# NorthStarUAS/ImageAnalysis

Measured on AMD Instinct MI355X. Metric: image_pairs_matched_per_sec, higher is better.
Workload: dtype u8 (int8 MFMA, int32 accumulate)

## Files before the change

### imageanalysis_amd/csrc/match_knn2sym.hip

```cpp
#include "iamx_common.h"
#include "sym_cand_rule.h"

namespace {

typedef int v4i __attribute__((ext_vector_type(4)));
typedef int v2i __attribute__((ext_vector_type(2)));
typedef int v16i __attribute__((ext_vector_type(16)));
typedef unsigned v2u __attribute__((ext_vector_type(2)));

#ifndef IAMX_DESC_OFFSET
#define IAMX_DESC_OFFSET 128
#endif
constexpr int D = IAMX_DESC_DIM;
constexpr int CHUNK = 128;
constexpr int BIG = 0x3F000000;

struct Pack3Args {
    const void *src;
    const int64_t *src_off;
    int64_t single_n;
    const int32_t *dst_off;
    int8_t *dst;
    int32_t *sn2, *sct, *sperm, *sinv;
    int32_t *n2, *nb, *pos;
// ... 650 lines not shown
#pragma unroll
        for (int k = 0; k < 8; ++k) load_op(0, 0, k, aop[0], tbop[0]);
#pragma unroll
        for (int k = 0; k < 8 / PP; ++k) load_op(0, 1, k, aop[1], tbop[1]);
        issue(0, 0, accs[0][0], accs[0][1]);
        __builtin_amdgcn_sched_barrier(0);
        int rbo = 0, rbo_prev = 2 * NW * CHUNK;
        const int wave_u = uniform32(wave);
        typedef __attribute__((address_space(3))) const int8_t *lds_bytes;
        int opoff[4], tboff = 2 * CHUNK * D + 16 * g;
#pragma unroll
        for (int s = 0; s < 4; ++s) opoff[s] = c * D + (((2 * s + g) ^ ((c >> 1) & 7)) * 16);
        auto load_op_at = [&](int tile, int k, v4i (&a)[4], v4i (&tbv)[4]) {
            if (k < 4) tbv[k] = *reinterpret_cast<const __attribute__((address_space(3))) v4i *>((lds_bytes)lds + tboff + tile * 128 + 32 * k);
            else a[k - 4] = *reinterpret_cast<const __attribute__((address_space(3))) v4i *>((lds_bytes)lds + opoff[k - 4] + tile * (32 * D));
        };
        const unsigned stage_voff = (unsigned)((tid >> 3) * D + (((tid & 7) ^ ((tid >> 4) & 7)) * 16));
        const unsigned lds_tile_at = (unsigned)(uintptr_t)(lds_ptr)(lds_tile + wave_u * (64 * 16));
        const unsigned lds_tb_at = (unsigned)(uintptr_t)(lds_ptr)(lds_tb + (wave_u & (CHUNK / 64 - 1)) * 64);
        const unsigned ct_voff = (unsigned)((tid & (CHUNK - 1)) * 4);
#if defined(IAMX_T_STAMPS)
        const unsigned long long loop_c0 = __builtin_amdgcn_s_memtime(), loop_r0 = __builtin_amdgcn_s_memrealtime();
        __builtin_amdgcn_s_waitcnt(0xC07F);
#endif
        for (int ch = 0; ch < nchunks; ++ch) {
            const int buf = ch & 1;
            if constexpr (PP == 4) {
            constexpr int BAR = (NT4 - 1) * PP - 1;
            static_assert(NW == 4 && PIECES == 4 && BAR + 4 < NS && (NT / 8) % 16 == 0, "the gaps below are form 2's");
            const int chs = ch + 2 < nchunks ? ch + 2 : nchunks - 1;
            const int8_t *const sg_tile = tbase + (int64_t)chs * (CHUNK * D);
            const int8_t *const sg_ct = reinterpret_cast<const int8_t *>(tci + chs * CHUNK);
            int mR[NW], mL = BIG, mU1 = BIG, mU2 = BIG;
            static_for<0, NS>([&](auto st_c) {
                constexpr int st = decltype(st_c)::value;
                constexpr int t = st / PP, ph = st % PP, qp = 2 * ph, cur = st & 1;
                constexpr int nst = st + 1 < NS ? st + 1 : 0;
#if defined(IAMX_T_STAMPS)
                unsigned long long stamp_t0 = 0, stamp_t1 = 0;
                if constexpr (IAMX_T_STAMPS == st + 1 || (st == BAR && IAMX_T_STAMPS == 17)) SWEEP_STAMP(stamp_t0);
                if constexpr (st == 0 && IAMX_T_STAMPS == 19) {
                    SWEEP_STAMP(stamp_t0);
                    SWEEP_STAMP(stamp_t1);
                    stamp_sum += stamp_t1 - stamp_t0;
                }
#endif
                if constexpr (st == BAR) {
                    __builtin_amdgcn_s_waitcnt(0x0070);
#if defined(IAMX_T_STAMPS)
                    if constexpr (IAMX_T_STAMPS == 17) {
                        SWEEP_STAMP(stamp_t1);
                        stamp_sum += stamp_t1 - stamp_t0;
                    }
                    if constexpr (IAMX_T_STAMPS == 18) SWEEP_STAMP(stamp_t0);
#endif
                    __syncthreads();
#if defined(IAMX_T_STAMPS)
                    if constexpr (IAMX_T_STAMPS == 18) {
                        SWEEP_STAMP(stamp_t1);
                        stamp_sum += stamp_t1 - stamp_t0;
                    }
#endif
                }
                issue(nst / PP, 2 * (nst % PP), accs[cur ^ 1][0], accs[cur ^ 1][1], false);
                auto operand_reads = [&]() {
                    static_for<(st == BAR - 1 ? 1 : 0), (st == BAR - 2 ? 2 : 1)>([&](auto d_c) {
                        constexpr int sr = st + decltype(d_c)::value;
                        constexpr int T = (sr + 1) / PP + 1, i = (sr + 1) % PP;
#pragma unroll
                        for (int k = i * 8 / PP; k < (i + 1) * 8 / PP; ++k) load_op_at(T % NT4, k, aop[T & 1], tbop[T & 1]);
                    });
                };
                if constexpr (st == BAR) {
#pragma unroll
                    for (int s = 0; s < 4; ++s) opoff[s] ^= CHUNK * D;
                    tboff ^= CHUNK * 4;
                }
                constexpr int nv = (ph == 2 ? 36 : ph == 3 ? 40 : 32) + (st == BAR + 2 ? 11 : 0) + (st == BAR + 3 ? 5 : 0) +
                                   (st >= BAR && st <= BAR + PIECES ? 1 : 0) +
                                   (st == NS - 1 ? 2 : 0);
                constexpr int tail = (st == BAR - 1 ? 0 : st == BAR - 2 ? 4 : 2) + (ph == 3 ? 1 + 2 : 0) +
                                     (st == BAR + 1 ? 2 : 0) + (st == BAR + 3 ? 1 : 0);
                constexpr bool staging = st >= BAR && st <= BAR + PIECES;
                constexpr int STAGE_GAP = 1, STAGE_AT = 8 + 1;
                constexpr int blk_at = sweep_gap_valu(nv, tail, true, 0) + sweep_gap_valu(nv, tail, true, 1) +
                                       sweep_gap_valu(nv, tail, true, 2) - (staging ? 2 : 0);
                static_assert(ph == 3 || (blk_at >= 6 && blk_at < 31), "gaps 3 and 4 hold the last two minima of column chain 0");
                const v16i acc0 = accs[cur][0], acc1 = accs[cur][1];
                int (&rc_)[16] = r[t & 1];
                int (&rp)[16] = r[(t + 1) & 1];
                static_for<0, 32>([&](auto i_c) {
                    constexpr int i = decltype(i_c)::value, op = sweep_min_order(ph < 3, blk_at, i);
                    if constexpr (op < 16) {
                        rc_[op] = qp == 0 ? min(acc0[op], acc1[op]) : min(min(rc_[op], acc0[op]), acc1[op]);
                    } else {
                        constexpr int w = op - 16;
                        int &mm = m[qp + (w >> 3)][t & 3];
                        const v16i &acc = w < 8 ? acc0 : acc1;
                        mm = min(min(mm, acc[2 * (w & 7)]), acc[2 * (w & 7) + 1]);
                        if constexpr (ph < 3 && i == blk_at) row_min16_block<2 * ph, true>(rp, mm);
                        if constexpr (ph < 3 && i == blk_at + 1) row_min16_block<2 * ph + 1, true>(rp, mm);
                        if constexpr (staging && w == STAGE_AT) {
                            if constexpr (st < BAR + PIECES)
                                stage_piece_held<16>(sg_tile + (st - BAR) * ((NT / 8) * D) + stage_voff,
                                                     lds_tile_at + buf * (CHUNK * D) + (st - BAR) * NT * 16, mm);
                            else
                                stage_piece_held<4>(sg_ct + ct_voff, lds_tb_at + buf * (CHUNK * 4), mm);
                        }
                    }
                });
                pin_accs(accs[cur ^ 1][0], accs[cur ^ 1][1]);
                operand_reads();
                if constexpr (ph == 2) {
#pragma unroll
                    for (int k = 0; k < 4; ++k) bu[k] = rp[4 * k] + lo_lane;
                }
                if constexpr (ph == 3) {
                    int *const dst = row_dst + (t > 0 ? rbo : rbo_prev) + (t > 0 ? t - 1 : NT4 - 1) * 32;
                    row_min16_piece<3>(rp, bu, lo_lane, dst);
                }
                if constexpr (st == BAR + 1) {
#pragma unroll
                    for (int w = 0; w < NW; ++w) mR[w] = lds_row[rbo_prev + w * CHUNK + mrow];
                }
                if constexpr (st == BAR + 2) {
#pragma unroll
                    for (int w = 0; w < NW; ++w) {
                        const int uw = mR[w] + spread_w[w];
                        mL = min(mL, mR[w]);
                        mU2 = min(max(mU1, uw), mU2);
                        mU1 = min(mU1, uw);
                    }
                }
                if constexpr (st == BAR + 3)
                    __builtin_amdgcn_raw_buffer_store_b64(v2i{mL, pack_row_bounds(mL, mU1, mU2)}, rowp_rsrc,
                                                          merger && ch > 0 ? ((ch - 1) * CHUNK + mrow) * 8 : RANGE_DROP, 0, 0);
                static_for<0, 8>([&](auto g_c) {
                    constexpr int g = decltype(g_c)::value;
                    __builtin_amdgcn_sched_group_barrier(0x008, 1, 0);
                    __builtin_amdgcn_sched_group_barrier(0x002, sweep_gap_valu(nv, tail, ph < 3, g) + (g == 7 ? 3 : 0) -
                                                                    (staging && g == STAGE_GAP ? 1 : 0), 0);
                });
                __builtin_amdgcn_sched_barrier(0);
#if defined(IAMX_T_STAMPS)
                if constexpr (IAMX_T_STAMPS == st + 1) {
                    SWEEP_STAMP(stamp_t1);
                    stamp_sum += stamp_t1 - stamp_t0;
                }
#endif
            });
            } else {
#pragma unroll
            for (int st = 0; st < NS; ++st) {
                const int t = st / PP, qp = 2 * (st % PP), cur = st & 1;
                if (st == (NT4 - 1) * PP - 1) {
                    __builtin_amdgcn_s_waitcnt(0x0070);
                    __syncthreads();
                    stage_direct(ch + 2 < nchunks ? ch + 2 : nchunks - 1, buf);
                    merge_rows(ch - 1, rbo_prev, merger && ch > 0);
                }
                if (st + 1 < NS) issue((st + 1) / PP, 2 * ((st + 1) % PP), accs[cur ^ 1][0], accs[cur ^ 1][1]);
                else issue(0, 0, accs[cur ^ 1][0], accs[cur ^ 1][1]);
                {
                    const int T = (st + 1) / PP + 1, i = (st + 1) % PP;
#pragma unroll
                    for (int k = i * 8 / PP; k < (i + 1) * 8 / PP; ++k)
                        load_op(T < NT4 ? buf : buf ^ 1, T % NT4, k, aop[T & 1], tbop[T & 1]);
                }
                const v16i acc0 = accs[cur][0], acc1 = accs[cur][1];
                int t0 = min(min(m[qp][t & 3], acc0[0]), acc0[1]);
                int t1m = min(min(m[qp + 1][t & 3], acc1[0]), acc1[1]);
#pragma unroll
                for (int reg = 2; reg < 16; reg += 2) {
                    t0 = min(min(t0, acc0[reg]), acc0[reg + 1]);
                    t1m = min(min(t1m, acc1[reg]), acc1[reg + 1]);
                }
                m[qp][t & 3] = t0;
                m[qp + 1][t & 3] = t1m;
                int (&rc_)[16] = r[t & 1];
                if (qp == 0) {
#pragma unroll
                    for (int reg = 0; reg < 16; ++reg) rc_[reg] = min(acc0[reg], acc1[reg]);
                } else {
#pragma unroll
                    for (int reg = 0; reg < 16; ++reg) rc_[reg] = min(min(rc_[reg], acc0[reg]), acc1[reg]);
                }
                {
                    int (&rp)[16] = r[(t + 1) & 1];
                    const int tp = t > 0 ? t - 1 : NT4 - 1;
                    int *dst = row_dst + (t > 0 ? rbo : rbo_prev) + tp * 32;
                    if constexpr (PP == 1) {
                        int m0, m1;
                        half_wave_min16<true>(rp, lo_lane, m0, m1);
                        dst[0] = m0;
                        dst[16] = m1;
                    } else {
                        if (0 * PP / 4 == st % PP) row_min16_piece<0>(rp, bu, lo_lane, dst);
                        if (1 * PP / 4 == st % PP) row_min16_piece<1>(rp, bu, lo_lane, dst);
                        if (2 * PP / 4 == st % PP) row_min16_piece<2>(rp, bu, lo_lane, dst);
                        if (3 * PP / 4 == st % PP) row_min16_piece<3>(rp, bu, lo_lane, dst);
                    }
                }
#pragma unroll
                for (int i = 0; i < 8; ++i) {
                    __builtin_amdgcn_sched_group_barrier(0x008, 1, 0);
                    __builtin_amdgcn_sched_group_barrier(0x002, PIPE, 0);
                }
                __builtin_amdgcn_sched_barrier(0);
            }
            }
            rbo_prev = rbo;
            rbo = rbo == 2 * NW * CHUNK ? 0 : rbo + NW * CHUNK;
        }
#if defined(IAMX_T_STAMPS)
        if constexpr (PP == 4) {
            unsigned long long loop_c1;
            SWEEP_STAMP(loop_c1);
            stamp_cycles += loop_c1 - loop_c0;
            stamp_ticks += __builtin_amdgcn_s_memrealtime() - loop_r0;
            stamp_chunks += (unsigned)nchunks;
            if (A.stamps && lane == 0) {
                unsigned long long *o = A.stamps + ((size_t)blockIdx.x * NW + wave) * 4;
                o[0] = stamp_sum;
                o[1] = stamp_chunks;
                o[2] = stamp_cycles;
                o[3] = stamp_ticks;
            }
        }
#endif
        int64_t col_v = 0;
        if constexpr (ITEMS) col_v = A.col_off[u];
        {
            int m0, m1;
            half_wave_min16<true>(r[(NT4 - 1) & 1], lo_lane, m0, m1);
            int *dst = row_dst + rbo_prev + (NT4 - 1) * 32;
            dst[0] = m0;
            dst[16] = m1;
        }
        wait_direct();
        __syncthreads();
        merge_rows(nchunks - 1, rbo_prev, merger);

        const int64_t col_u = ITEMS ? uniform64(col_v) : 0;
        if (wave_valid) {
            unsigned ownpack = 0;
            int v1s[QW], v2s[QW];
#pragma unroll
            for (int qb = 0; qb < QW; ++qb) {
                const int lo01 = min(m[qb][0], m[qb][1]), hi01 = max(m[qb][0], m[qb][1]);
                const int lo23 = min(m[qb][2], m[qb][3]), hi23 = max(m[qb][2], m[qb][3]);
                const int a1 = min(lo01, lo23), a2 = min(max(lo01, lo23), min(hi01, hi23));
                const int b1 = __shfl_xor(a1, 32), b2 = __shfl_xor(a2, 32);
                const int v1 = min(a1, b1), v2 = min(max(a1, b1), min(a2, b2));
                v1s[qb] = v1;
                v2s[qb] = v2;
#if !defined(IAMX_T_NOMASK)
                const unsigned own = (m[qb][0] <= v2 ? 1u : 0u) | (m[qb][1] <= v2 ? 2u : 0u) |
                                     (m[qb][2] <= v2 ? 4u : 0u) | (m[qb][3] <= v2 ? 8u : 0u);
                ownpack |= own << (4 * qb);
#endif
            }
            const unsigned othpack = A.colmask ? (unsigned)__shfl_xor((int)ownpack, 32) : 0u;
            const int row0 = q0 + QW * rc;
            if (g == 0) {
#pragma unroll
                for (int qb = 0; qb < QW; ++qb)
                    if (row0 + qb < nb)
                        *reinterpret_cast<v2i *>(A.col + 2 * ((ITEMS ? col_u : A.col_off[u]) + row0 + qb)) = v2i{v1s[qb], v2s[qb]};
                if (A.colmask) {
                    uint8_t *dst = A.colmask + (ITEMS ? col_u : A.col_off[u]) + row0;
                    if (QW == 8 && row0 + QW <= nb) {
                        auto spread = [](unsigned nib4) {
                            const unsigned x = (nib4 | (nib4 << 8)) & 0x00FF00FFu;
                            return (x | (x << 4)) & 0x0F0F0F0Fu;
                        };
                        const unsigned lo = spread(ownpack & 0xFFFFu) | (spread(othpack & 0xFFFFu) << 4);
                        const unsigned hi = spread(ownpack >> 16) | (spread(othpack >> 16) << 4);
                        *reinterpret_cast<v2u *>(dst) = v2u{lo, hi};
                    } else {
#pragma unroll
                        for (int qb = 0; qb < QW; ++qb)
                            if (row0 + qb < nb)
                                dst[qb] = (uint8_t)(((ownpack >> (4 * qb)) & 15u) | (((othpack >> (4 * qb)) & 15u) << 4));
                    }
                }
            }
        }
        if constexpr (!ITEMS) break;
        else if (++u == uniform32(u_end)) break;
    }
}

constexpr int sweep16_gap_valu(int nv, int g) { return nv / 8 + (g < nv % 8 ? 1 : 0); }

constexpr int SWEEP16_RAW_COMBO = 256 + 32;
constexpr int SWEEP16_RAW_CHUNK = (CHUNK / 16) * 4 * SWEEP16_RAW_COMBO;
constexpr int SWEEP16_LDS_FORM2 = 2 * CHUNK * D + 2 * CHUNK * 4 + 3 * 4 * CHUNK * 4 + 2 * 4 * 4 + (2 * 4 * CHUNK + 4 * 256) * 4;
constexpr int SWEEP16_LDS_BYTES = SWEEP16_LDS_FORM2 + 4 * 2 * SWEEP16_RAW_CHUNK;
static_assert(SWEEP16_LDS_FORM2 % 16 == 0 && SWEEP16_LDS_BYTES <= 160 * 1024, "aligned, and inside a compute unit's LDS");

template <int PIPE>
__global__ __launch_bounds__(256, 1) void knn2sym16_kernel(SymArgs A)
{
    constexpr int NW = 4, QB = 16, WGROWS = NW * QB * 16, NT = NW * 64;
    constexpr int PIECES = CHUNK * D / 16 / NT;
    constexpr int NT16 = CHUNK / 16, SPT = 4, QS = QB / SPT, NS = NT16 * SPT;
    static_assert(WGROWS == 1024 && PIECES == 4 && NS == 32 && D == 128, "form 2's workgroup");
    extern __shared__ __attribute__((aligned(16))) int8_t lds[];
    int8_t *lds_tile = lds;
    int *lds_tb = reinterpret_cast<int *>(lds + 2 * CHUNK * D);
    int *lds_row = lds_tb + 2 * CHUNK;
    int *lds_cq = lds_row + 3 * NW * CHUNK;
    int *lds_dump = lds_cq + 2 * NW;
    const int tid = threadIdx.x, lane = tid & 63, wave = tid >> 6;
    const int n = lane & 15, lg = lane >> 4;
    const int rn = ((n & 7) << 1) | (n >> 3);

    int vid;
    {
        const int total = A.total_wg, bid = blockIdx.x;
        const int xcd = bid & 7, k = bid >> 3, q = total >> 3, r = total & 7;
        vid = (xcd < r ? xcd * (q + 1) : r * (q + 1) + (xcd - r) * q) + k;
    }
    int u = A.wg_off[3 * vid], u_end = u + A.wg_off[3 * vid + 1], item_wgi = A.wg_off[3 * vid + 2];
    v4i bq[QB][2];
    int fl[4];
    int bimg_held = -1;
    asm volatile("" : "+v"(u_end), "+v"(item_wgi), "+v"(bimg_held));
    const int raw_wave = SWEEP16_LDS_FORM2 + wave * (2 * SWEEP16_RAW_CHUNK);
    const int raw_wr = raw_wave + lg * SWEEP16_RAW_COMBO + n * 16;
    const int raw_rd = raw_wave + (lane >> 1) * SWEEP16_RAW_COMBO + (lane & 1) * 16;
#if defined(IAMX_T_STAMPS)
    unsigned long long stamp_chunks = 0, stamp_cycles = 0, stamp_ticks = 0, stamp_tail = 0, stamp_c1 = 0;
#endif
    int nx_b = A.upairs[2 * u], nx_a = A.upairs[2 * u + 1];
    int nx_boff = A.img_off[nx_b], nx_nb = A.img_n[nx_b], nx_aoff = A.img_off[nx_a], nx_na = A.img_n[nx_a];
    int64_t nx_rowp = A.rowp_off[u];
    for (;;) {
        const int bimg = uniform32(nx_b);
        const int boff = uniform32(nx_boff), nb = uniform32(nx_nb);
        const int aoff = uniform32(nx_aoff), na = uniform32(nx_na);
        const int capA = (na + CHUNK - 1) / CHUNK * CHUNK;
        const int nchunks = capA / CHUNK;
        const int wgi = uniform32(item_wgi);
        const int q0 = wgi * WGROWS + wave * (QB * 16);
        const bool wave_valid = q0 < nb;
        const int64_t rbase = uniform64(nx_rowp) + (int64_t)wgi * capA;
        if (uniform32(bimg_held) >= 0) __syncthreads();

        if (bimg != uniform32(bimg_held)) {
            bimg_held = bimg;
#pragma unroll
            for (int qb = 0; qb < QB; ++qb) {
                int row = q0 + QB * rn + qb;
                row = row < nb ? row : nb - 1;
                const v4i *src = reinterpret_cast<const v4i *>(A.sdesc + (int64_t)(boff + row) * D);
#pragma unroll
                for (int s = 0; s < 2; ++s) {
                    bq[qb][s] = ~src[4 * s + lg];
                    asm volatile("" : "+a"(bq[qb][s]));
                }
            }
            {
                int spread = 0;
                if (wave_valid) {
                    const int g_lo = rn & ~1, g_hi = rn | 1;
                    const int r_lo = q0 + QB * g_lo < nb ? q0 + QB * g_lo : nb - 1;
                    const int r_hi = q0 + QB * g_hi + QB - 1 < nb ? q0 + QB * g_hi + QB - 1 : nb - 1;
                    spread = (A.sn2[boff + r_hi] >> 1) - (A.sn2[boff + r_lo] >> 1);
                }
#pragma unroll
                for (int sh = 32; sh >= 1; sh >>= 1) spread = max(spread, __shfl_xor(spread, sh));
                if (lane == 0) lds_cq[wave] = spread;
            }
#pragma unroll
            for (int j = 0; j < 4; ++j) {
                const int r_lo = q0 + 2 * QB * (2 * j + (lane & 1));
                fl[j] = wave_valid ? A.sn2[boff + (r_lo < nb ? r_lo : nb - 1)] >> 1 : 0;
            }
        }
        if (!wave_valid) {
#pragma unroll
            for (int k = 0; k < 3 * CHUNK / 64; ++k)
                lds_row[((k / (CHUNK / 64)) * NW + wave) * CHUNK + (k % (CHUNK / 64)) * 64 + lane] = BIG;
        }
        int m[QB][4];
#pragma unroll
        for (int qb = 0; qb < QB; ++qb)
#pragma unroll
            for (int k = 0; k < 4; ++k) m[qb][k] = BIG;

        const int8_t *tbase = A.sdesc + (int64_t)aoff * D;
        const int32_t *tci = A.sct + aoff;
        typedef __attribute__((address_space(3))) void *lds_ptr;
        auto stage_direct = [&](int ch, int buf) {
#pragma unroll
            for (int j = 0; j < PIECES; ++j) {
                const int e = j * NT + tid, row = e >> 3, slot = (e & 7) ^ ((row >> 1) & 7);
                const int8_t *gsrc = tbase + (int64_t)(ch * CHUNK + row) * D + slot * 16;
                int8_t *ldst = lds_tile + buf * (CHUNK * D) + (j * NT + wave * 64) * 16;
                __builtin_amdgcn_global_load_lds(gsrc, (lds_ptr)ldst, 16, 0, 0);
            }
            __builtin_amdgcn_global_load_lds(tci + ch * CHUNK + (tid & (CHUNK - 1)),
                                             (lds_ptr)(lds_tb + buf * CHUNK + (wave & (CHUNK / 64 - 1)) * 64), 4, 0, 0);
        };
        auto wait_direct = [&]() { __builtin_amdgcn_s_waitcnt(0x0F70); };
        const int mrow = (wave & 1) * 64 + lane;
        const bool merger = wave < 2;
        constexpr int RSRC_WORD3_DATA_FORMAT_32 = 4 << 15;
        constexpr int RANGE_DROP = 0x7FFFFFF0;
        const __amdgpu_buffer_rsrc_t rowp_rsrc =
            __builtin_amdgcn_make_buffer_rsrc(A.rowp + 2 * rbase, (short)0, capA * 8, RSRC_WORD3_DATA_FORMAT_32);
        int spread_w[NW];
        auto merge_rows = [&](int ch, int rbo, bool store) {
            int L = BIG, U1 = BIG, U2 = BIG;
#pragma unroll
            for (int w = 0; w < NW; ++w) {
                const int R = lds_row[rbo + w * CHUNK + mrow];
                const int uw = R + spread_w[w];
                L = min(L, R);
                U2 = min(max(U1, uw), U2);
                U1 = min(U1, uw);
            }
            __builtin_amdgcn_raw_buffer_store_b64(v2i{L, pack_row_bounds(L, U1, U2)}, rowp_rsrc,
                                                  store ? (ch * CHUNK + mrow) * 8 : RANGE_DROP, 0, 0);
        };

        int *const row_dst = (lane & 1) == 0 && wave_valid
            ? lds_row + wave * CHUNK + 4 * (lane >> 1)
            : lds_dump + wave * 256 + 4 * lane;
        typedef __attribute__((address_space(3))) int8_t *lds_wbytes;
        typedef __attribute__((address_space(3))) v4i *lds_v4i;
        auto raw_write = [&](int at, int tile, const int (&rr)[4]) {
            *reinterpret_cast<lds_v4i>((lds_wbytes)lds + at + tile * (4 * SWEEP16_RAW_COMBO)) = v4i{rr[0], rr[1], rr[2], rr[3]};
        };
        auto raw_read = [&](int at, int j, v4i (&v)[2]) {
#pragma unroll
            for (int hi = 0; hi < 2; ++hi)
                v[hi] = *reinterpret_cast<lds_v4i>((lds_wbytes)lds + at + j * 32 + hi * 128);
        };
        auto raw_group = [&](int j, const v4i (&v)[2], int (&x)[4]) {
#pragma unroll
            for (int i = 0; i < 4; ++i) x[i] = min(v[0][i], v[1][i]) + fl[j];
        };
        auto raw_store = [&](int rbo_at, int (&x)[4]) {
#pragma unroll
            for (int i = 0; i < 4; ++i) x[i] = min(x[i], __builtin_amdgcn_update_dpp(0, x[i], 0xB1, 0xF, 0xF, true));
            *reinterpret_cast<v4i *>(row_dst + rbo_at) = v4i{x[0], x[1], x[2], x[3]};
        };
        v4i aop[2][2], ct[2];
        v4i accs[2][QS];
        int r[2][4];
#pragma unroll
        for (int k = 0; k < 4; ++k) r[1][k] = BIG;

        {
            const int un = u + 1 < u_end ? u + 1 : u;
            nx_b = A.upairs[2 * un];
            nx_a = A.upairs[2 * un + 1];
            nx_rowp = A.rowp_off[un];
        }
        stage_direct(0, 0);
        stage_direct(nchunks > 1 ? 1 : 0, 1);
        wait_direct();
        __syncthreads();
#pragma unroll
        for (int w = 0; w < NW; ++w) spread_w[w] = __builtin_amdgcn_readfirstlane(lds_cq[w]);
        {
            const int b = uniform32(nx_b), a = uniform32(nx_a);
            nx_boff = A.img_off[b];
            nx_nb = A.img_n[b];
            nx_aoff = A.img_off[a];
            nx_na = A.img_n[a];
        }
        typedef __attribute__((address_space(3))) const int8_t *lds_bytes;
        int opoff[2], tboff = 2 * CHUNK * D + 16 * lg;
#pragma unroll
        for (int s = 0; s < 2; ++s) opoff[s] = n * D + (((4 * s + lg) ^ ((n >> 1) & 7)) * 16);
        auto load_ops = [&](int tile, v4i (&a)[2], v4i &c) {
            c = *reinterpret_cast<const __attribute__((address_space(3))) v4i *>((lds_bytes)lds + tboff + tile * 64);
#pragma unroll
            for (int s = 0; s < 2; ++s)
                a[s] = *reinterpret_cast<const __attribute__((address_space(3))) v4i *>((lds_bytes)lds + opoff[s] + tile * (16 * D));
        };
        auto issue = [&](auto tp_c, auto qp_c, v4i (&acc)[QS]) {
            constexpr int tp = decltype(tp_c)::value, qp = decltype(qp_c)::value;
#pragma unroll
            for (int j = 0; j < QS; ++j) acc[j] = __builtin_amdgcn_mfma_i32_16x16x64_i8(aop[tp][0], bq[qp + j][0], ct[tp], 0, 0, 0);
#pragma unroll
            for (int j = 0; j < QS; ++j) acc[j] = __builtin_amdgcn_mfma_i32_16x16x64_i8(aop[tp][1], bq[qp + j][1], acc[j], 0, 0, 0);
        };
        load_ops(0, aop[0], ct[0]);
        load_ops(1, aop[1], ct[1]);
        issue(int_c<0>{}, int_c<0>{}, accs[0]);
        __builtin_amdgcn_sched_barrier(0);
        int rbo = 0, rbo_prev = 2 * NW * CHUNK;
        const int wave_u = uniform32(wave);
        const unsigned stage_voff = (unsigned)((tid >> 3) * D + (((tid & 7) ^ ((tid >> 4) & 7)) * 16));
        const unsigned lds_tile_at = (unsigned)(uintptr_t)(lds_ptr)(lds_tile + wave_u * (64 * 16));
        const unsigned lds_tb_at = (unsigned)(uintptr_t)(lds_ptr)(lds_tb + (wave_u & (CHUNK / 64 - 1)) * 64);
        const unsigned ct_voff = (unsigned)((tid & (CHUNK - 1)) * 4);
#if defined(IAMX_T_STAMPS)
        const unsigned long long loop_c0 = __builtin_amdgcn_s_memtime(), loop_r0 = __builtin_amdgcn_s_memrealtime();
        __builtin_amdgcn_s_waitcnt(0xC07F);
        if (stamp_c1) stamp_tail += loop_c0 - stamp_c1;
#endif
        auto chunk = [&](int ch, auto stage_c) __attribute__((always_inline)) {
            constexpr bool STAGE = decltype(stage_c)::value != 0;
            const int buf = ch & 1;
            constexpr int BAR = (NT16 - 2) * SPT;
            static_assert(BAR + PIECES < NS, "the stage's five pieces fit behind the barrier");
            const int8_t *const sg_tile = tbase + (int64_t)(ch + 2) * (CHUNK * D);
            const int8_t *const sg_ct = reinterpret_cast<const int8_t *>(tci + (ch + 2) * CHUNK);
            const int raw_cur = buf * SWEEP16_RAW_CHUNK, raw_prev = SWEEP16_RAW_CHUNK - raw_cur;
            const int wr_cur = raw_wr + raw_cur, wr_prev = raw_wr + raw_prev, rd_prev = raw_rd + raw_prev;
            int mR[NW], mL = BIG, mU1 = BIG, mU2 = BIG;
            constexpr int RSTORE = 4 * SPT + 1;
            static_assert(RSTORE < BAR, "the rows are stored in front of the barrier");
            v4i rdv[2];
            int racc[4], rx[4], rh[4];
            static_for<0, NS>([&](auto st_c) {
                constexpr int st = decltype(st_c)::value;
                constexpr int t = st / SPT, ph = st % SPT, qp = QS * ph, cur = st & 1, kk = (t >> 1) & 3;
                constexpr int nst = st + 1 < NS ? st + 1 : 0;
                constexpr bool staging = STAGE && st >= BAR && st <= BAR + PIECES;
                if constexpr (st == BAR) {
                    __builtin_amdgcn_s_waitcnt(0x0070);
                    __syncthreads();
                }
                issue(int_c<(nst / SPT) & 1>{}, int_c<QS * (nst % SPT)>{}, accs[cur ^ 1]);
#pragma unroll
                for (int j = 0; j < QS; ++j) {
                    const v4i &a = accs[cur][j];
                    int &mm = m[qp + j][kk];
                    mm = min(min(mm, a[0]), a[1]);
                    if constexpr (staging) {
                        if (j == 1) {
                            if constexpr (st < BAR + PIECES)
                                stage_piece_held<16>(sg_tile + (st - BAR) * ((NT / 8) * D) + stage_voff,
                                                     lds_tile_at + buf * (CHUNK * D) + (st - BAR) * NT * 16, mm);
                            else
                                stage_piece_held<4>(sg_ct + ct_voff, lds_tb_at + buf * (CHUNK * 4), mm);
                        }
                    }
                    mm = min(min(mm, a[2]), a[3]);
                }
                const v4i a0 = accs[cur][0], a1 = accs[cur][1], a2 = accs[cur][2], a3 = accs[cur][3];
                int (&rc_)[4] = r[t & 1];
#pragma unroll
                for (int i = 0; i < 4; ++i)
                    rc_[i] = ph == 0 ? min(min(min(a0[i], a1[i]), a2[i]), a3[i])
                                     : min(min(min(min(rc_[i], a0[i]), a1[i]), a2[i]), a3[i]);
                if constexpr (ph == 0) raw_write(t > 0 ? wr_cur : wr_prev, t > 0 ? t - 1 : NT16 - 1, r[(t + 1) & 1]);
                if constexpr (ph == 0 && t < 4) raw_read(rd_prev, t, rdv);
                if constexpr (ph == 2 && t < 4) {
                    if constexpr (t == 0) raw_group(0, rdv, racc);
                    else raw_group(t, rdv, rx);
                    if constexpr (t == 1) {
#pragma unroll
                        for (int i = 0; i < 4; ++i) racc[i] = min(racc[i], rx[i]);
                    }
                    if constexpr (t == 2) {
#pragma unroll
                        for (int i = 0; i < 4; ++i) rh[i] = rx[i];
                    }
                    if constexpr (t == 3) {
#pragma unroll
                        for (int i = 0; i < 4; ++i) racc[i] = min(min(racc[i], rh[i]), rx[i]);
                    }
                }
                if constexpr (st == RSTORE) raw_store(rbo_prev, racc);
                if constexpr (ph == SPT - 1) {
                    if constexpr (t + 2 == NT16) {
#pragma unroll
                        for (int s = 0; s < 2; ++s) opoff[s] ^= CHUNK * D;
                        tboff ^= CHUNK * 4;
                    }
                    load_ops((t + 2) % NT16, aop[t & 1], ct[t & 1]);
                }
                if constexpr (st == BAR + 1) {
#pragma unroll
                    for (int w = 0; w < NW; ++w) mR[w] = lds_row[rbo_prev + w * CHUNK + mrow];
                }
                if constexpr (st == BAR + 2) {
#pragma unroll
                    for (int w = 0; w < NW; ++w) {
                        const int uw = mR[w] + spread_w[w];
                        mL = min(mL, mR[w]);
                        mU2 = min(max(mU1, uw), mU2);
                        mU1 = min(mU1, uw);
                    }
                    asm volatile("" : "+v"(mL), "+v"(mU1), "+v"(mU2));
                }
                if constexpr (st == BAR + 3)
                    __builtin_amdgcn_raw_buffer_store_b64(v2i{mL, pack_row_bounds(mL, mU1, mU2)}, rowp_rsrc,
                                                          merger && ch > 0 ? ((ch - 1) * CHUNK + mrow) * 8 : RANGE_DROP, 0, 0);
                constexpr int nv = 16 + (ph == 2 && t < 4 ? (t & 1 ? 12 : 8) : 0) + (st == RSTORE ? 4 : 0) + (st == 0 ? 3 : 0) +
                                   (staging ? 2 : 0) + (st == BAR + 2 ? 11 : 0) + (st == BAR + 3 ? 5 : 0) +
                                   (st == NS - 1 ? 2 : 0) + (PIPE - 2);
                static_for<0, 8>([&](auto g_c) {
                    constexpr int g = decltype(g_c)::value;
                    __builtin_amdgcn_sched_group_barrier(0x008, 1, 0);
                    __builtin_amdgcn_sched_group_barrier(0x002, sweep16_gap_valu(nv, g) + (g == 7 ? 3 : 0), 0);
                });
                __builtin_amdgcn_sched_barrier(0);
            });
            rbo_prev = rbo;
            rbo = rbo == 2 * NW * CHUNK ? 0 : rbo + NW * CHUNK;
        };
        int ch = 0;
        for (; ch + 2 < nchunks; ++ch) chunk(ch, int_c<1>{});
        for (; ch < nchunks; ++ch) chunk(ch, int_c<0>{});
#if defined(IAMX_T_STAMPS)
        {
            unsigned long long loop_c1;
            SWEEP_STAMP(loop_c1);
            stamp_cycles += loop_c1 - loop_c0;
            stamp_ticks += __builtin_amdgcn_s_memrealtime() - loop_r0;
            stamp_chunks += (unsigned)nchunks;
            stamp_c1 = loop_c1;
            if (A.stamps && lane == 0) {
                unsigned long long *o = A.stamps + ((size_t)blockIdx.x * NW + wave) * 4;
                o[0] = stamp_tail;
                o[1] = stamp_chunks;
                o[2] = stamp_cycles;
                o[3] = stamp_ticks;
            }
        }
#endif
        const int64_t col_v = A.col_off[u];
        {
            const int last = ((nchunks - 1) & 1) * SWEEP16_RAW_CHUNK;
            raw_write(raw_wr + last, NT16 - 1, r[(NT16 - 1) & 1]);
            v4i v[4][2];
            int x[4][4];
#pragma unroll
            for (int j = 0; j < 4; ++j) raw_read(raw_rd + last, j, v[j]);
#pragma unroll
            for (int j = 0; j < 4; ++j) raw_group(j, v[j], x[j]);
#pragma unroll
            for (int i = 0; i < 4; ++i) x[0][i] = min(min(x[0][i], x[1][i]), min(x[2][i], x[3][i]));
            raw_store(rbo_prev, x[0]);
        }
        wait_direct();
        __syncthreads();
        merge_rows(nchunks - 1, rbo_prev, merger);

        const int64_t col_u = uniform64(col_v);
        if (wave_valid) {
            int mk[QB / 2][4], a1[QB / 2], a2[QB / 2];
#pragma unroll
            for (int j = 0; j < QB / 2; ++j) {
#pragma unroll
                for (int k = 0; k < 4; ++k) {
                    const v2u x = __builtin_amdgcn_permlane32_swap((unsigned)m[j][k], (unsigned)m[j + QB / 2][k], false, false);
                    mk[j][k] = min((int)x[0], (int)x[1]);
                }
                const int lo01 = min(mk[j][0], mk[j][1]), hi01 = max(mk[j][0], mk[j][1]);
                const int lo23 = min(mk[j][2], mk[j][3]), hi23 = max(mk[j][2], mk[j][3]);
                a1[j] = min(lo01, lo23);
                a2[j] = min(max(lo01, lo23), min(hi01, hi23));
            }
            int v1s[4], v2s[4];
#pragma unroll
            for (int p = 0; p < 4; ++p) {
                const v2u x1 = __builtin_amdgcn_permlane16_swap((unsigned)a1[p], (unsigned)a1[p + 4], false, false);
                const v2u x2 = __builtin_amdgcn_permlane16_swap((unsigned)a2[p], (unsigned)a2[p + 4], false, false);
                v1s[p] = min((int)x1[0], (int)x1[1]);
                v2s[p] = min(max((int)x1[0], (int)x1[1]), min((int)x2[0], (int)x2[1]));
            }
            const int row0 = q0 + QB * rn + 4 * lg;
            unsigned maskw = 0;
            if (A.colmask) {
                unsigned ownpack = 0;
#pragma unroll
                for (int p = 0; p < 4; ++p) {
                    const v2u w = __builtin_amdgcn_permlane16_swap((unsigned)v2s[p], (unsigned)v2s[p], false, false);
#pragma unroll
                    for (int c = 0; c < 2; ++c) {
                        const int j = p + 4 * c, v2 = (int)w[c];
                        const unsigned own = (mk[j][0] <= v2 ? 1u : 0u) | (mk[j][1] <= v2 ? 2u : 0u) |
                                             (mk[j][2] <= v2 ? 4u : 0u) | (mk[j][3] <= v2 ? 8u : 0u);
                        ownpack |= own << (4 * j);
                    }
                }
                const v2u g = __builtin_amdgcn_permlane16_swap(ownpack, ownpack, false, false);
                auto spread = [](unsigned nib4) {
                    const unsigned x = (nib4 | (nib4 << 8)) & 0x00FF00FFu;
                    return (x | (x << 4)) & 0x0F0F0F0Fu;
                };
                const int sh = 16 * (lg & 1);
                maskw = spread((g[0] >> sh) & 0xFFFFu) | (spread((g[1] >> sh) & 0xFFFFu) << 4);
            }
            int32_t *const cdst = A.col + 2 * (col_u + row0);
            if (row0 + 4 <= nb) {
                *reinterpret_cast<v4i *>(cdst) = v4i{v1s[0], v2s[0], v1s[1], v2s[1]};
                *reinterpret_cast<v4i *>(cdst + 4) = v4i{v1s[2], v2s[2], v1s[3], v2s[3]};
                if (A.colmask) *reinterpret_cast<unsigned *>(A.colmask + col_u + row0) = maskw;
            } else {
#pragma unroll
                for (int p = 0; p < 4; ++p)
                    if (row0 + p < nb) {
                        *reinterpret_cast<v2i *>(cdst + 2 * p) = v2i{v1s[p], v2s[p]};
                        if (A.colmask) A.colmask[col_u + row0 + p] = (uint8_t)(maskw >> (8 * p));
                    }
            }
        }
        if (++u == uniform32(u_end)) break;
    }
}

struct NarTask { int p, cls, item0, n; };
struct NarLayout {
    int64_t ctl, pair_base, mask, slot, items, res, tasks, total;
    int64_t item_cap, task_cap;
};
__host__ __device__ inline NarLayout narrow_layout(int64_t rows, int64_t n_pairs)
{
    NarLayout L;
    auto up = [](int64_t v) { return (v + 255) / 256 * 256; };
    L.item_cap = rows;
    L.task_cap = rows / 64 + 80 * n_pairs + 64;
    int64_t o = 0;
    L.ctl = o;        o += 256;
    L.pair_base = o;  o += up(n_pairs * 4);
    L.mask = o;       o += up(rows * 8);
    L.slot = o;       o += up(rows * 8);
    L.items = o;      o += up(L.item_cap * 8);
    L.res = o;        o += up(L.item_cap * 16);
    L.tasks = o;      o += up(L.task_cap * 16);
    L.total = o;
    return L;
}
constexpr int NAR_MIN_TRAIN = 1024;
constexpr int NAR_ITEMS = 256;

struct CandArgs {
    const int32_t *sn2, *sperm, *img_off, *img_n;
    const int32_t *pairs;
    const int32_t *osrc;
    const int32_t *wg_off;
    const int64_t *col_off, *rowp_off, *out_off;
    const int32_t *col, *rowp;
    double thresh;
    double K;
    uint8_t *keep;
    int32_t *cand_cnt;
    int32_t *cand_q;
    int32_t *task_total;
    int32_t *tasks;
    int32_t *d2;
    int wg_shift;
    const uint8_t *colmask;
    int8_t *nar;
    int64_t rows_total;
    int n_pairs, wgrows;
};

constexpr int CAND_ROWS = 4;

template <int NW>
__device__ __forceinline__ void cand_merge_partials(const int32_t *__restrict__ rowq, int64_t cap, int (&L)[CAND_ROWS],
                                                    int (&U1)[CAND_ROWS], int (&U2)[CAND_ROWS])
{
    v4i e[NW][2];
#pragma unroll
    for (int w = 0; w < NW; ++w) {
        e[w][0] = *reinterpret_cast<const v4i *>(rowq + 2 * (w * cap));
        e[w][1] = *reinterpret_cast<const v4i *>(rowq + 2 * (w * cap) + 4);
    }
#pragma unroll
    for (int w = 0; w < NW; ++w)
#pragma unroll
        for (int i = 0; i < CAND_ROWS; ++i) {
            int eL, e1, e2;
            unpack_row_bounds(v2i{e[w][i >> 1][2 * (i & 1)], e[w][i >> 1][2 * (i & 1) + 1]}, eL, e1, e2);
            L[i] = min(L[i], eL);
            const int n1 = min(U1[i], e1);
            U2[i] = min(max(U1[i], e1), min(U2[i], e2));
            U1[i] = n1;
        }
}

__device__ __forceinline__ void symcand_rows_pair(const CandArgs &A, int p, int pos0)
{
    const int qimg = uniform32(A.pairs[2 * p]);
    const int u = uniform32(A.osrc[2 * p]), role = uniform32(A.osrc[2 * p + 1]);
    const int soff = uniform32(A.img_off[qimg]), n = uniform32(A.img_n[qimg]);
    if ((int)blockIdx.x * (256 * CAND_ROWS) >= n) return;
    const bool in = pos0 < n;
    const int64_t cap = (n + CHUNK - 1) / CHUNK * CHUNK;
    const int nwg = uniform32(A.wg_off[u + 1]) - uniform32(A.wg_off[u]);
    const int64_t ob = uniform64(A.out_off[p]);
    const int64_t cb = uniform64(A.col_off[u]);
    const int32_t *rowq = A.rowp + 2 * uniform64(A.rowp_off[u]);
    int U2[CAND_ROWS];
    long long Lb[CAND_ROWS], Ub[CAND_ROWS];
    v4i n2 = {0, 0, 0, 0};
    if (in) n2 = *reinterpret_cast<const v4i *>(A.sn2 + soff + pos0);
    if (role == 0) {
        v4i c[2] = {{0, 0, 0, 0}, {0, 0, 0, 0}};
        if (in) {
            c[0] = *reinterpret_cast<const v4i *>(A.col + 2 * (cb + pos0));
            c[1] = *reinterpret_cast<const v4i *>(A.col + 2 * (cb + pos0) + 4);
        }
#pragma unroll
        for (int i = 0; i < CAND_ROWS; ++i) {
            const int par = n2[i] & 1;
            const long long cq = n2[i] >> 1;
            U2[i] = 0x7FFFFFFF;
            Lb[i] = 2 * (c[i >> 1][2 * (i & 1)] + cq) + par;
            Ub[i] = 2 * (c[i >> 1][2 * (i & 1) + 1] + cq) + par + 1;
        }
    } else {
        int L[CAND_ROWS], U1[CAND_ROWS];
#pragma unroll
        for (int i = 0; i < CAND_ROWS; ++i) L[i] = U1[i] = U2[i] = 0x7FFFFFFF;
        if (in) {
            const int32_t *rq = rowq + 2 * pos0;
            switch (nwg) {
            case 1: cand_merge_partials<1>(rq, cap, L, U1, U2); break;
            case 2: cand_merge_partials<2>(rq, cap, L, U1, U2); break;
            case 3: cand_merge_partials<3>(rq, cap, L, U1, U2); break;
            case 4: cand_merge_partials<4>(rq, cap, L, U1, U2); break;
            default: {
                int w = 0;
                for (; w + 4 <= nwg; w += 4) cand_merge_partials<4>(rq + 2 * (w * cap), cap, L, U1, U2);
                for (; w < nwg; ++w) cand_merge_partials<1>(rq + 2 * (w * cap), cap, L, U1, U2);
            }
            }
        }
#pragma unroll
        for (int i = 0; i < CAND_ROWS; ++i) {
            const int par = n2[i] & 1;
            Lb[i] = 2ll * L[i] + par;
            Ub[i] = 2ll * U2[i] + par + 1;
        }
    }
    unsigned kbits = 0u;
#pragma unroll
    for (int i = 0; i < CAND_ROWS; ++i) {
        if (Lb[i] < 0) Lb[i] = 0;
        if (pos0 + i < n && !sym_cand_reject(Lb[i], Ub[i], A.K) && sym_cand_keep(Lb[i], Ub[i], A.thresh))
            kbits |= 1u << i;
    }
    if (kbits == 0u) return;
    const unsigned long long holders = __ballot(1);
    int wave_cnt = 0;
#pragma unroll
    for (int i = 0; i < CAND_ROWS; ++i) wave_cnt += __popcll(__ballot((kbits >> i) & 1u));
    if ((int)(threadIdx.x & 63) == __ffsll((long long)holders) - 1) atomicAdd(A.cand_cnt + p, wave_cnt);
    const int ncls = role == 0 ? 8 : nwg;
    const bool nar_ok = A.nar != nullptr && A.img_n[A.pairs[2 * p + 1]] >= NAR_MIN_TRAIN && ncls <= 64;
#pragma unroll
    for (int i = 0; i < CAND_ROWS; ++i) {
        if (!((kbits >> i) & 1u)) continue;
        const int pos = pos0 + i;
        const int orig = A.sperm[soff + pos];
        atomicOr(reinterpret_cast<unsigned *>(A.keep) + ((ob + orig) >> 5), 1u << ((ob + orig) & 31));
        A.d2[2 * (ob + orig) + 1] = (int)(Ub[i] < 0x7FFFFFFFll ? Ub[i] : 0x7FFFFFFFll);
        if (nar_ok) {
            unsigned long long mk = 0ull;
            if (role == 0) {
                mk = A.colmask[cb + pos];
            } else {
                for (int w = 0; w < nwg; ++w)
                    if (rowq[2 * (w * cap + pos)] <= U2[i]) mk |= 1ull << w;
            }
            const NarLayout NL = narrow_layout(A.rows_total, A.n_pairs);
            reinterpret_cast<unsigned long long *>(A.nar + NL.mask)[ob + orig] = mk;
        }
    }
}

__global__ __launch_bounds__(256) void symcand_rows_kernel(CandArgs A)
{
    for (int p = blockIdx.y; p < A.n_pairs; p += gridDim.y)
        symcand_rows_pair(A, p, ((int)blockIdx.x * 256 + (int)threadIdx.x) * CAND_ROWS);
}

__global__ __launch_bounds__(256) void symcand_clear_kernel(unsigned *keep, int64_t n_words, int32_t *cand_cnt, int n_pairs)
{
    const int64_t stride = (int64_t)gridDim.x * 256;
    for (int64_t i = (int64_t)blockIdx.x * 256 + threadIdx.x; i < n_words; i += stride) keep[i] = 0u;
    for (int64_t i = (int64_t)blockIdx.x * 256 + threadIdx.x; i < n_pairs; i += stride) cand_cnt[i] = 0;
}

__global__ __launch_bounds__(256) void symcand_kernel(CandArgs A)
{
    __shared__ int wcnt[4];
    __shared__ int s_base;
    const int p = blockIdx.x;
    const NarLayout NL = narrow_layout(A.rows_total, A.n_pairs);
    if (A.cand_cnt[p] == 0) {
        if (threadIdx.x == 0) {
            A.cand_cnt[p] = 0;
            if (A.nar != nullptr) reinterpret_cast<int32_t *>(A.nar + NL.pair_base)[p] = -1;
        }
        return;
    }
    const int qimg = A.pairs[2 * p];
    const int u = A.osrc[2 * p], role = A.osrc[2 * p + 1];
    const int n = A.img_n[qimg];
    const int nwg = A.wg_off[u + 1] - A.wg_off[u];
    const int64_t ob = A.out_off[p];
    const int ncls = role == 0 ? 8 : nwg;
    const bool nar_ok = A.nar != nullptr && A.img_n[A.pairs[2 * p + 1]] >= NAR_MIN_TRAIN && ncls <= 64;
    unsigned long long *maskv = reinterpret_cast<unsigned long long *>(A.nar + NL.mask);
    const int lane = threadIdx.x & 63, wave = threadIdx.x >> 6;
    const unsigned *keepw = reinterpret_cast<const unsigned *>(A.keep);
    const int64_t w_first = ob >> 5, w_last = (ob + n - 1) >> 5;
    int out = 0;
    for (int64_t wbase = w_first; wbase <= w_last; wbase += 256) {
        const int64_t w = wbase + threadIdx.x;
        unsigned bits = 0u;
        if (w <= w_last) {
            bits = keepw[w];
            if (w == w_first) bits &= ~0u << (ob & 31);
            if (w == w_last) bits &= ~0u >> (31 - (int)((ob + n - 1) & 31));
        }
        const int c = __popc(bits);
        int x = c;
#pragma unroll
        for (int sft = 1; sft < 64; sft <<= 1) {
            const int y = __shfl_up(x, sft);
            if (lane >= sft) x += y;
        }
        if (lane == 63) wcnt[wave] = x;
        __syncthreads();
        int woff = 0, tot = 0;
#pragma unroll
        for (int k = 0; k < 4; ++k) {
            if (k < wave) woff += wcnt[k];
            tot += wcnt[k];
        }
        int at = out + woff + x - c;
        const int row0 = (int)((w << 5) - ob);
        for (unsigned b = bits; b; b &= b - 1) A.cand_q[ob + at++] = row0 + __ffs((int)b) - 1;
        out += tot;
        __syncthreads();
    }
    bool narrow = nar_ok && out > 64;
    if (A.nar != nullptr) {
        __shared__ int cls_cnt[64], cls_off[65], cls_task[65], s_nb;
        int32_t *ctl = reinterpret_cast<int32_t *>(A.nar + NL.ctl);
        int32_t *pair_base = reinterpret_cast<int32_t *>(A.nar + NL.pair_base);
        v2i *slot = reinterpret_cast<v2i *>(A.nar + NL.slot);
        v2i *items = reinterpret_cast<v2i *>(A.nar + NL.items);
        NarTask *ntasks = reinterpret_cast<NarTask *>(A.nar + NL.tasks);
        if (narrow) {
            if (threadIdx.x < 64) cls_cnt[threadIdx.x] = 0;
            __syncthreads();
            int run = 0;
            for (int base = 0; base < out; base += 256) {
                const int i = base + threadIdx.x;
                unsigned long long mk = 0ull;
                if (i < out) mk = maskv[ob + A.cand_q[ob + i]];
                const int nk = __popcll(mk);
                int x = nk;
#pragma unroll
                for (int sft = 1; sft < 64; sft <<= 1) {
                    const int y = __shfl_up(x, sft);
                    if (lane >= sft) x += y;
                }
                if (lane == 63) wcnt[wave] = x;
                __syncthreads();
                int woff = 0, tot = 0;
#pragma unroll
                for (int w = 0; w < 4; ++w) {
                    if (w < wave) woff += wcnt[w];
                    tot += wcnt[w];
                }
                if (i < out) {
                    slot[ob + i] = v2i{run + woff + x - nk, nk};
                    for (unsigned long long b = mk; b; b &= b - 1) atomicAdd(&cls_cnt[__ffsll((long long)b) - 1], 1);
                }
                run += tot;
                __syncthreads();
            }
            if (threadIdx.x == 0) {
                int o = 0, nt = 0;
                for (int cidx = 0; cidx < 64; ++cidx) {
                    cls_off[cidx] = o;
                    cls_task[cidx] = nt;
                    o += cls_cnt[cidx];
                    nt += (cls_cnt[cidx] + NAR_ITEMS - 1) / NAR_ITEMS;
                }
                cls_off[64] = o;
                cls_task[64] = nt;
                const int b0 = atomicAdd(ctl + 1, run);
                bool ok = (int64_t)b0 + run <= NL.item_cap;
                int t0 = 0;
                if (ok) {
                    t0 = atomicAdd(ctl + 0, nt);
                    ok = (int64_t)t0 + nt <= NL.task_cap;
                }
                s_nb = ok ? b0 : -1;
                s_base = t0;
                pair_base[p] = ok ? b0 : -1;
            }
            __syncthreads();
            narrow = s_nb >= 0;
            if (narrow) {
                const int b0 = s_nb, t0 = s_base;
                if (threadIdx.x < 64) {
                    const int cidx = threadIdx.x, cnt_c = cls_cnt[cidx];
                    for (int t = 0; t * NAR_ITEMS < cnt_c; ++t)
                        ntasks[t0 + cls_task[cidx] + t] =
                            NarTask{p, cidx, b0 + cls_off[cidx] + t * NAR_ITEMS, min(NAR_ITEMS, cnt_c - t * NAR_ITEMS)};
                }
                __syncthreads();
                if (threadIdx.x < 64) cls_cnt[threadIdx.x] = 0;
// ... 559 lines not shown
                                bd2[h] = min(bd2[h], d1k);
                            }
                        } else {
#pragma unroll
                            for (int reg = 0; reg < 16; ++reg) {
                                const int dk = 2 * acc[reg] + ((tk[reg >> 2][reg & 3] >> 4) & 1);
                                const int ik = s_idx[buf][j * 32 + 8 * (reg >> 2) + 4 * g + (reg & 3)];
                                if (dk < bd1[h] || (dk == bd1[h] && ik < bi1[h])) {
                                    bd2[h] = bd1[h];
                                    bd1[h] = dk;
                                    bi1[h] = ik;
                                } else {
                                    bd2[h] = min(bd2[h], dk);
                                }
                            }
                        }
                    }
                }
            }
            if (ph + 1 < nph) stage(buf ^ 1, pre, pre_meta);
            __syncthreads();
        }
#pragma unroll
        for (int h = 0; h < 2; ++h) {
            const int od1 = __shfl_xor(bd1[h], 32), oi1 = __shfl_xor(bi1[h], 32), od2 = __shfl_xor(bd2[h], 32);
            int f_d, f_i, s_d;
            if (od1 < bd1[h] || (od1 == bd1[h] && oi1 < bi1[h])) {
                f_d = od1; f_i = oi1;
                s_d = min(bd1[h], od2);
            } else {
                f_d = bd1[h]; f_i = bi1[h];
                s_d = min(od1, bd2[h]);
            }
            if (g == 0 && live[h] && (h == 0 || n_sets == 2)) res[slot[h]] = v4i{f_d, f_i, s_d, 0};
        }
    }
}

__device__ __forceinline__ void narrow_finish_pair(const NarArgs &A, int p)
{
    const NarLayout NL = narrow_layout(A.rows_total, A.n_pairs);
    const int32_t *pair_base = reinterpret_cast<const int32_t *>(A.nar + NL.pair_base);
    const v2i *slot = reinterpret_cast<const v2i *>(A.nar + NL.slot);
    const v4i *res = reinterpret_cast<const v4i *>(A.nar + NL.res);
    if (p == 0 && threadIdx.x == 0) {
        int32_t *ctl = reinterpret_cast<int32_t *>(A.nar + NL.ctl);
        ctl[0] = ctl[1] = ctl[2] = 0;
    }
    const int b0 = pair_base[p];
    if (b0 < 0) return;
    const int64_t cb = A.out_off[p];
    const int cnt = A.cand_cnt[p];
    const int qoff = A.img_off[A.pairs[2 * p]];
    for (int k = threadIdx.x; k < cnt; k += 256) {
        const v2i sl = slot[cb + k];
        int f_d = NAR_D_INVALID, f_i = NAR_D_INVALID, s_d = NAR_D_INVALID;
        for (int j = 0; j < sl.y; ++j) {
            const v4i e = res[b0 + sl.x + j];
            if (e.x < f_d || (e.x == f_d && e.y < f_i)) {
                s_d = min(f_d, e.z);
                f_d = e.x;
                f_i = e.y;
            } else {
                s_d = min(s_d, e.x);
            }
        }
        const int q = A.cand_q[cb + k];
        if (f_d >= (1 << 26) || s_d >= (1 << 26)) {
            atomicAdd(A.zero_div + 1, 1);
            A.cand_t[cb + k] = 0;
            A.cand_metric[cb + k] = 0.0;
            A.cand_keep[cb + k] = 0;
            continue;
        }
        const int na = A.norm_q[qoff + q];
        const int d1 = f_d + na, d2 = s_d + na;
        *reinterpret_cast<v2i *>(A.d2w + 2 * (cb + q)) = v2i{d1, d2};
        const float f0 = (float)sqrt((double)d1);
        const float f1 = (float)sqrt((double)d2);
        double mt;
        bool ok = false;
        if (f1 == 0.0f) {
            mt = __longlong_as_double(0x7FF8000000000000LL);
            atomicAdd(A.zero_div, 1);
        } else {
            mt = (double)f0 * ((double)f0 / (double)f1);
            ok = mt < A.thresh;
        }
        A.cand_t[cb + k] = f_i;
        A.cand_metric[cb + k] = mt;
        A.cand_keep[cb + k] = ok ? 1 : 0;
    }
}

__global__ __launch_bounds__(256) void symcompact_kernel(const int64_t *cand_off,
                                                         const int32_t *cand_cnt,
                                                         const uint8_t *cand_keep,
                                                         int32_t *q, int32_t *t,
                                                         double *metric,
                                                         int32_t *surv_cnt,
                                                         int32_t *task_total, NarArgs N)
{
    __shared__ int wcnt[4];
    const int p = blockIdx.x;
    if (cand_cnt[p] == 0) {
        if (threadIdx.x == 0) {
            surv_cnt[p] = 0;
            if (p == 0) {
                task_total[0] = task_total[1] = 0;
                if (N.nar != nullptr) {
                    int32_t *ctl = reinterpret_cast<int32_t *>(N.nar + narrow_layout(N.rows_total, N.n_pairs).ctl);
                    ctl[0] = ctl[1] = ctl[2] = 0;
                }
            }
        }
        return;
    }
    if (N.nar != nullptr) {
        narrow_finish_pair(N, p);
        __threadfence_block();
        __syncthreads();
    }
    const int64_t b = cand_off[p];
    const int cnt = cand_cnt[p];
    const int lane = threadIdx.x & 63, wave = threadIdx.x >> 6;
    int out = 0;
    for (int base = 0; base < cnt; base += 256) {
        const int i = base + threadIdx.x;
        const bool k = i < cnt && cand_keep[b + i];
        int vq = 0, vt = 0;
        double vm = 0.0;
        if (k) { vq = q[b + i]; vt = t[b + i]; vm = metric[b + i]; }
        const unsigned long long mask = __ballot(k);
        const int before = __popcll(mask & ((1ull << lane) - 1ull));
        if (lane == 0) wcnt[wave] = __popcll(mask);
        __syncthreads();
        int woff = 0, tot = 0;
#pragma unroll
        for (int w = 0; w < 4; ++w) {
            if (w < wave) woff += wcnt[w];
            tot += wcnt[w];
        }
        if (k) {
            const int64_t o = b + out + woff + before;
            q[o] = vq; t[o] = vt; metric[o] = vm;
        }
        out += tot;
        __syncthreads();
    }
    if (threadIdx.x == 0) {
        surv_cnt[p] = out;
        if (p == 0) task_total[0] = task_total[1] = 0;
    }
}

}

extern "C" int64_t iamx_desc3_rows_cap(int64_t n_rows)
{
    if (n_rows <= 0) return 0;
    return (n_rows + CHUNK - 1) / CHUNK * CHUNK;
}

extern "C" int iamx_knn2sym_rows_per_wg(int form)
{
    return form == 2 ? 1024 : (form == 1 ? 512 : (form == 0 ? 256 : 0));
}

template <typename SRC>
static int pack3_launch(Pack3Args P, int64_t total_rows, int max_rows, void *stream, const char *what)
{
    hipStream_t st = iamx::as_stream(stream);
    if (total_rows <= 0 || max_rows <= 0) return IAMX_OK;
    const int cap = (max_rows + CHUNK - 1) / CHUNK * CHUNK;
    hipLaunchKernelGGL(pack3_rows_kernel<SRC>, dim3((unsigned)((total_rows * 8 + 255) / 256)),
                       dim3(256), 0, st, P, total_rows);
    const int64_t groups = (int64_t)((max_rows + 255) / 256) * P.n_img;
    int split = 1;
    while (split < 32 && groups * split < 2048 && max_rows > 1024 * split) split *= 2;
    if (split > 1) (void)hipMemsetAsync(P.pos, 0, (size_t)total_rows * sizeof(int32_t), st);
    hipLaunchKernelGGL(pack3_rank_bins_kernel, dim3((unsigned)P.n_img), dim3(1024), 0, st, P);
    hipLaunchKernelGGL(pack3_rank_kernel,
                       dim3((unsigned)((max_rows + 255) / 256), (unsigned)P.n_img, (unsigned)split),
                       dim3(256), 0, st, P);
    hipLaunchKernelGGL(pack3_scatter_kernel<SRC>,
                       dim3((unsigned)(((int64_t)cap * 8 + 255) / 256), (unsigned)P.n_img),
                       dim3(256), 0, st, P);
    return iamx::check_launch(what);
}

template <typename SRC>
static int pack3_single(const SRC *src, int64_t n_rows, int8_t *dst, int32_t *sn2, int32_t *sct,
                        int32_t *sperm, int32_t *sinv, int32_t *scratch, void *stream,
                        const char *what)
{
    if (n_rows < 0 || n_rows > (1 << 24) || (n_rows > 0 && !src) || !dst || !sn2 || !sct || !sperm ||
        !sinv || !scratch)
        return iamx::fail(IAMX_EINVAL, "%s: null pointer or bad row count", what);
    Pack3Args P{src, nullptr, n_rows, nullptr, dst, sn2, sct, sperm, sinv,
                scratch, scratch + n_rows, scratch + 2 * n_rows, 1};
    return pack3_launch<SRC>(P, n_rows, (int)n_rows, stream, what);
}

extern "C" int iamx_desc3_pack_u8(const uint8_t *src, int64_t n_rows, int8_t *dst, int32_t *sn2,
                                  int32_t *sct, int32_t *sperm, int32_t *sinv, int32_t *scratch,
                                  void *stream)
{
    return pack3_single(src, n_rows, dst, sn2, sct, sperm, sinv, scratch, stream, "iamx_desc3_pack_u8");
}

extern "C" int iamx_desc3_pack_f32(const float *src, int64_t n_rows, int8_t *dst, int32_t *sn2,
                                   int32_t *sct, int32_t *sperm, int32_t *sinv, int32_t *scratch,
                                   void *stream)
{
    return pack3_single(src, n_rows, dst, sn2, sct, sperm, sinv, scratch, stream, "iamx_desc3_pack_f32");
}

extern "C" int iamx_desc3_pack_batch_u8(const uint8_t *src, const int64_t *src_off,
                                        const int32_t *dst_off, int n_img, int64_t total_rows,
                                        int max_rows_per_image, int8_t *dst, int32_t *sn2,
                                        int32_t *sct, int32_t *sperm, int32_t *sinv,
                                        int32_t *scratch, void *stream)
{
    IAMX_REQUIRE(src && src_off && dst_off && dst && sn2 && sct && sperm && sinv && scratch,
                 "null pointer");
    IAMX_REQUIRE(n_img > 0 && total_rows >= 0 && max_rows_per_image >= 0, "bad count");
    Pack3Args P{src, src_off, 0, dst_off, dst, sn2, sct, sperm, sinv,
                scratch, scratch + total_rows, scratch + 2 * total_rows, n_img};
    return pack3_launch<uint8_t>(P, total_rows, max_rows_per_image, stream, "iamx_desc3_pack_batch_u8");
}

#define SWEEP_FORM2 8, 4, 0, 5, 2, 0, true, 128, 1
#define SWEEP_FORM1 4, 4, 0, 6, 2, 0, true, 128, 2
#define SWEEP_FORM0 2, 4, 0, 6, 2, 0, true, 128, 2
#define SWEEP_ITEMS2 8, 4, 1, 5, 2, 0, true, 128, 1
#define SWEEP_STR2(...) #__VA_ARGS__
#define SWEEP_STR(...) SWEEP_STR2(__VA_ARGS__)

#if defined(IAMX_T_STAMPS)
static unsigned long long *g_sweep_stamps = nullptr;
extern "C" int iamx_knn2sym_set_stamps(void *buf)
{
    g_sweep_stamps = static_cast<unsigned long long *>(buf);
    return IAMX_OK;
}
#define SWEEP_STAMPS_ARG , g_sweep_stamps
#else
#define SWEEP_STAMPS_ARG
#endif

extern "C" const char *iamx_knn2sym_kernel_id(int form)
{
    switch (form) {
    case 2: return "knn2sym_kernel<" SWEEP_STR(SWEEP_ITEMS2) ">";
    case 1: return "knn2sym_kernel<" SWEEP_STR(SWEEP_FORM1) ">";
    case 0: return "knn2sym_kernel<" SWEEP_STR(SWEEP_FORM0) ">";
    default: return "";
    }
}

extern "C" int iamx_knn2sym_sweep(const int8_t *sdesc, const int32_t *sn2, const int32_t *sct,
                                  const int32_t *img_off, const int32_t *img_n,
                                  const int32_t *upairs, const int32_t *wg_off,
                                  const int64_t *col_off, const int64_t *rowp_off, int n_u,
                                  int total_wg, int form, int32_t *col, int32_t *rowp,
                                  uint8_t *colmask, void *stream)
{
    IAMX_REQUIRE(sdesc && sn2 && sct && img_off && img_n && upairs && wg_off && col_off && rowp_off &&
                     col && rowp,
                 "null pointer");
    IAMX_REQUIRE(n_u >= 0 && total_wg >= 0, "negative count");
    IAMX_REQUIRE(form >= 0 && form <= 2, "form must be 0 (256 rows), 1 (512) or 2 (1024)");
    if (n_u == 0 || total_wg == 0) return IAMX_OK;
    SymArgs a{sdesc, sn2, sct, img_off, img_n, upairs, wg_off, col_off, rowp_off, col, rowp, n_u, total_wg,
              colmask SWEEP_STAMPS_ARG};
    const dim3 g((unsigned)total_wg);
    hipStream_t st = iamx::as_stream(stream);
    if (form == 2) hipLaunchKernelGGL((knn2sym_kernel<SWEEP_FORM2>), g, dim3(256), 0, st, a);
    else if (form == 1) hipLaunchKernelGGL((knn2sym_kernel<SWEEP_FORM1>), g, dim3(256), 0, st, a);
    else hipLaunchKernelGGL((knn2sym_kernel<SWEEP_FORM0>), g, dim3(256), 0, st, a);
    return iamx::check_launch("iamx_knn2sym_sweep");
}

extern "C" int iamx_knn2sym_sweep_items(const int8_t *sdesc, const int32_t *sn2, const int32_t *sct,
                                        const int32_t *img_off, const int32_t *img_n,
                                        const int32_t *upairs, const int32_t *items,
                                        const int64_t *col_off, const int64_t *rowp_off, int n_u,
                                        int n_items, int32_t *col, int32_t *rowp, uint8_t *colmask,
                                        void *stream)
{
    IAMX_REQUIRE(sdesc && sn2 && sct && img_off && img_n && upairs && items && col_off && rowp_off &&
                     col && rowp,
                 "null pointer");
    IAMX_REQUIRE(n_u >= 0 && n_items >= 0, "negative count");
    if (n_u == 0 || n_items == 0) return IAMX_OK;
    SymArgs a{sdesc, sn2, sct, img_off, img_n, upairs, items, col_off, rowp_off, col, rowp, n_u, n_items,
              colmask SWEEP_STAMPS_ARG};
    hipLaunchKernelGGL((knn2sym_kernel<SWEEP_ITEMS2>), dim3((unsigned)n_items), dim3(256), 0,
                       iamx::as_stream(stream), a);
    return iamx::check_launch("iamx_knn2sym_sweep_items");
}

#define SWEEP16_PIPE 2
extern "C" const char *iamx_knn2sym_items16_kernel_id(void)
{
    return "knn2sym16_kernel<" SWEEP_STR(SWEEP16_PIPE) ">";
}

extern "C" int iamx_knn2sym_sweep_items16(const int8_t *sdesc, const int32_t *sn2, const int32_t *sct,
                                          const int32_t *img_off, const int32_t *img_n,
                                          const int32_t *upairs, const int32_t *items,
                                          const int64_t *col_off, const int64_t *rowp_off, int n_u,
                                          int n_items, int32_t *col, int32_t *rowp, uint8_t *colmask,
                                          void *stream)
{
    IAMX_REQUIRE(sdesc && sn2 && sct && img_off && img_n && upairs && items && col_off && rowp_off &&
                     col && rowp,
                 "null pointer");
    IAMX_REQUIRE(n_u >= 0 && n_items >= 0, "negative count");
    if (n_u == 0 || n_items == 0) return IAMX_OK;
    SymArgs a{sdesc, sn2, sct, img_off, img_n, upairs, items, col_off, rowp_off, col, rowp, n_u, n_items,
              colmask SWEEP_STAMPS_ARG};
    static thread_local int raised_dev = -1;
    int dev = 0;
    if (hipGetDevice(&dev) != hipSuccess)
        return iamx::fail(IAMX_ELAUNCH, "iamx_knn2sym_sweep_items16: no current device");
    if (dev != raised_dev) {
        const hipError_t e = hipFuncSetAttribute(reinterpret_cast<const void *>(&knn2sym16_kernel<SWEEP16_PIPE>),
                                                 hipFuncAttributeMaxDynamicSharedMemorySize, SWEEP16_LDS_BYTES);
        if (e != hipSuccess)
            return iamx::fail(IAMX_ELAUNCH, "iamx_knn2sym_sweep_items16: dynamic LDS: %s", hipGetErrorString(e));
        raised_dev = dev;
    }
    hipLaunchKernelGGL((knn2sym16_kernel<SWEEP16_PIPE>), dim3((unsigned)n_items), dim3(256), SWEEP16_LDS_BYTES,
                       iamx::as_stream(stream), a);
    return iamx::check_launch("iamx_knn2sym_sweep_items16");
}

static bool narrow_enabled()
{
    const char *e = getenv("IAMX_EXACT_NARROW");
    return !(e && e[0] == '0');
}

extern "C" int64_t iamx_knn2sym_narrow_bytes(int64_t rows, int n_pairs)
{
    if (rows <= 0 || n_pairs <= 0) return 0;
    return narrow_layout(rows, n_pairs).total;
}

extern "C" int iamx_knn2sym_candidates(const int32_t *sn2, const int32_t *sperm,
                                       const int32_t *img_off, const int32_t *img_n,
                                       const int32_t *pairs, const int32_t *osrc,
                                       const int32_t *wg_off, const int64_t *col_off,
                                       const int64_t *rowp_off, const int64_t *out_off,
                                       const int32_t *col, const int32_t *rowp, int n_pairs,
                                       double thresh, uint8_t *keep, int32_t *cand_cnt,
                                       int32_t *cand_q, int32_t *task_total, int32_t *tasks,
                                       int32_t *d2, const uint8_t *colmask, void *nar,
                                       int64_t rows_total, int max_query_rows, int form, void *stream)
{
    IAMX_REQUIRE(sn2 && sperm && img_off && img_n && pairs && osrc && wg_off && col_off && rowp_off &&
                     out_off && col && rowp && keep && cand_cnt && cand_q && task_total && tasks && d2,
                 "null pointer");
    IAMX_REQUIRE(!nar || colmask, "narrow workspace without colmask");
    IAMX_REQUIRE(form >= 0 && form <= 2, "form must be 0, 1 or 2");
    if (n_pairs <= 0) return IAMX_OK;
    CandArgs a{sn2, sperm, img_off, img_n, pairs, osrc, wg_off, col_off, rowp_off, out_off, col, rowp,
               thresh, sym_cand_K(thresh), keep, cand_cnt, cand_q, task_total, tasks, d2, 8,
               colmask, narrow_enabled() ? static_cast<int8_t *>(nar) : nullptr, rows_total, n_pairs,
               iamx_knn2sym_rows_per_wg(form)};
    IAMX_REQUIRE(rows_total > 0 && rows_total < (1ll << 31), "rows_total = rows of all ordered pairs");
    IAMX_REQUIRE(max_query_rows > 0, "max_query_rows = rows of the largest query image");
    const int64_t keep_words = (rows_total + 31) / 32;
    const int64_t clear_wg = (keep_words + 4095) / 4096;
    hipLaunchKernelGGL(symcand_clear_kernel, dim3((unsigned)(clear_wg < 256 ? clear_wg : 256)), dim3(256), 0,
                       iamx::as_stream(stream), reinterpret_cast<unsigned *>(keep), keep_words, cand_cnt, n_pairs);
    hipLaunchKernelGGL(symcand_rows_kernel,
                       dim3((unsigned)((max_query_rows + 1023) / 1024), (unsigned)(n_pairs < 65535 ? n_pairs : 65535)),
                       dim3(256), 0, iamx::as_stream(stream), a);
    hipLaunchKernelGGL(symcand_kernel, dim3((unsigned)n_pairs), dim3(256), 0, iamx::as_stream(stream), a);
    return iamx::check_launch("iamx_knn2sym_candidates");
}

extern "C" int iamx_knn2sym_exact(const int8_t *desc, const int32_t *norm_q, const int32_t *norm_t,
                                  int32_t *key_t, int64_t total_rows,
                                  const int32_t *img_off, const int32_t *img_n, const int32_t *pairs,
                                  const int64_t *out_off, const int32_t *cand_cnt,
                                  int32_t *task_total, const int32_t *tasks, int32_t *cand_q,
                                  int n_pairs, double thresh, int32_t *d2, int32_t *cand_t,
                                  double *cand_metric, uint8_t *cand_keep, int32_t *surv_cnt,
                                  int32_t *zero_div, const int8_t *sdesc, const int32_t *sn2,
                                  const int32_t *sct, const int32_t *sperm, const int32_t *img_off3,
                                  const int32_t *osrc, void *nar, int64_t rows_total, int form,
                                  void *stream)
{
    IAMX_REQUIRE(desc && norm_q && norm_t && key_t && img_off && img_n && pairs && out_off && cand_cnt &&
                     task_total && tasks && cand_q && d2 && cand_t && cand_metric && cand_keep &&
                     surv_cnt && zero_div,
                 "null pointer");
    IAMX_REQUIRE(total_rows >= 0, "negative row count");
    if (n_pairs <= 0) return IAMX_OK;
    hipStream_t st = iamx::as_stream(stream);
    if (total_rows > 0) {
        int64_t gk = (total_rows + 255) / 256;
        hipLaunchKernelGGL(symexact_keys_kernel, dim3((unsigned)(gk > 4096 ? 4096 : gk)), dim3(256), 0, st,
                           norm_t, total_rows, key_t);
    }
    ExactArgs a{desc, norm_q, norm_t, key_t, n_pairs, img_off, img_n, pairs, out_off, cand_cnt, cand_q,
                task_total, tasks, thresh, d2, cand_t, cand_metric, cand_keep, zero_div};
    hipLaunchKernelGGL(symexact_kernel, dim3(1024), dim3(256), 0, st, a);
    const char *prune = getenv("IAMX_EXACT_PRUNE");
    if (prune && prune[0] == '0')
        hipLaunchKernelGGL((symexact_wg_kernel<false, 1>), dim3(2048), dim3(256), 0, st, a);
    else
        hipLaunchKernelGGL((symexact_wg_kernel<true, 2>), dim3(2048), dim3(256), 0, st, a);
    NarArgs nfin{};
    if (nar && narrow_enabled()) {
        if (!(sdesc && sn2 && sct && sperm && img_off3 && osrc && rows_total > 0 && form >= 0 && form <= 2))
            return iamx::fail(IAMX_EINVAL, "iamx_knn2sym_exact: narrow workspace without the sorted store");
        NarArgs na{desc, norm_q, img_off, pairs, osrc, out_off, cand_q, d2, sdesc, sn2, sct, sperm, img_off3,
                   img_n, static_cast<int8_t *>(nar), rows_total, n_pairs, iamx_knn2sym_rows_per_wg(form),
                   cand_cnt, thresh, d2, cand_t, cand_metric, cand_keep, zero_div};
        hipLaunchKernelGGL(symnarrow_kernel<3>, dim3(768), dim3(256), 0, st, na);
        nfin = na;
    }
    hipLaunchKernelGGL(symcompact_kernel, dim3((unsigned)n_pairs), dim3(256), 0, st, out_off,
                       cand_cnt, cand_keep, cand_q, cand_t, cand_metric, surv_cnt, task_total, nfin);
    return iamx::check_launch("iamx_knn2sym_exact");
}
```

### imageanalysis_amd/kernels.py

```python
import math
import os
import threading

import numpy as np
import torch

from . import _lib
from ._lib import check, lib, require_gpu, stream_ptr

I8, I32, I64, F64, U8 = torch.int8, torch.int32, torch.int64, torch.float64, torch.uint8
I16 = torch.int16


def _ptr(t):
    return _lib.c_void_p(t.data_ptr()) if t is not None else _lib.c_void_p(0)


def _dev(x, dtype):
    dev = require_gpu()
    if isinstance(x, torch.Tensor):
        return x.to(device=dev, dtype=dtype).contiguous()
    x = np.ascontiguousarray(x)
    if not x.flags.writeable:
        import warnings
# ... 754 lines not shown
    pts = torch.empty((max(cap, 1), 4), dtype=torch.float32, device=dev)
    rows = torch.empty((max(cap, 1), 2), dtype=I32, device=dev)
    flag = z32(2)
    work = torch.empty(n * (6 * stride + 2 * tab), dtype=I32, device=dev)
    slots = torch.empty((n, stride, 2), dtype=I32, device=dev)
    best = torch.from_numpy(np.tile(np.array([SMART_MIN_UNIQUE, 0], np.int32), (n, 1))).to(dev)
    improved, cnt, fit_status = z32(n), z32(n), z32(n)
    stats = z32(n, NB, 3)
    off = torch.zeros(n + 1, dtype=I64, device=dev)
    out_rows = torch.empty((max(total, 1), 2), dtype=I32, device=dev)
    active = torch.ones(n, dtype=I32, device=dev)
    act_h = np.ones(n, bool)
    while act_h.any() and (max_passes is None or len(res.stats) < max_passes):
        check(L.iamx_smart_stats(_ptr(idx), _ptr(d2), _ptr(row_off), _ptr(d_pairs), _ptr(kp_off), _ptr(xy),
                                 _ptr(size), _ptr(Hl), _ptr(active), n, float(match_ratio), float(min_pairs),
                                 cap, _ptr(bin_cnt), _ptr(seg_cnt), _ptr(seg_off), _ptr(pts), _ptr(rows),
                                 _ptr(flag), stream_ptr()), 'iamx_smart_stats')
        mask, model, _best, vstatus = verify_pairs(pts[:cap], seg_off, 'homography', float(tol),
                                                   hypotheses=hypotheses, seed=seed)
        check(L.iamx_smart_select(_ptr(d_pairs), _ptr(kp_off), _ptr(key2), _ptr(active), n, float(min_pairs),
                                  _ptr(bin_cnt), _ptr(seg_cnt), _ptr(seg_off), _ptr(pts), _ptr(rows),
                                  _ptr(mask), _ptr(vstatus), _ptr(model), cap, stride, tab, _ptr(work),
                                  _ptr(best), _ptr(improved), _ptr(slots), _ptr(cnt), _ptr(off),
                                  _ptr(out_rows), total, _ptr(stats), _ptr(Hl), _ptr(fit_status), _ptr(flag),
                                  stream_ptr()), 'iamx_smart_select')
        taken = improved.cpu().numpy()
        passes[live[act_h]] += 1
        st_h = np.full((P, NB, 3), -2, np.int32)
        st_h[live[act_h]] = stats.cpu().numpy()[act_h]
        tk_h = np.zeros(P, np.int32)
        tk_h[live] = taken
        res.stats.append(st_h)
        res.taken.append(tk_h)
        res.flag = flag.cpu().numpy()
        if res.flag.any():
            break
        act_h = taken > 0
        active.copy_(torch.from_numpy(act_h.astype(np.int32)))
    res.best[live] = best.cpu().numpy()
    if n == P:
        res.rows, res.off, res.cnt, res.H = out_rows, off, cnt, Hl.view(P, 3, 3)
        return res
    where = torch.from_numpy(live).to(dev)
    cnt_all[where] = cnt
    H[where] = Hl
    res.rows, res.cnt, res.H = out_rows, cnt_all, H.view(P, 3, 3)
    res.off = exclusive_scan(cnt_all)
    return res


BRUTE_DIST_BINS, BRUTE_ANGLE_BINS = 41, 21
BRUTE_CELLS = BRUTE_DIST_BINS * BRUTE_ANGLE_BINS
BRUTE_STEP_A = 2 * math.pi / (BRUTE_ANGLE_BINS - 1)
BRUTE_BATCH_BYTES = 4 << 30


class BruteResult(object):
    __slots__ = ('rows', 'off', 'cnt', 'chosen', 'stats', 'fit_cnt', 'bin_cnt', 'flag', 'slots', 'stride')

    def __init__(self, **kw):
        for k in self.__slots__:
            setattr(self, k, kw.get(k))


def brute_bytes(nq):
    nq = np.asarray(nq, np.int64).reshape(-1)
    if not len(nq):
        return 0
    stride = max(int(nq.max()), 1)
    return int(nq.sum()) * (32 + 25 * 9) + len(nq) * (32 * stride + 8 * _ratio_tab_size(stride) + 112 * BRUTE_CELLS)


def _brute_launch(store, pairs, kp_off, xy, size, key2, tol, min_pairs, match_ratio, step_d, hypotheses,
                  seed, flag):
    dev = require_gpu()
    L = lib()
    NC, P = BRUTE_CELLS, len(pairs)
    idx, d2, out_off = knn3_pairs(store, pairs)
    total = int(out_off[-1])
    nq = np.diff(out_off)
    stride = max(int(nq.max()), 1)
    tab = _ratio_tab_size(stride)
    cap = 9 * total
    d_pairs = torch.from_numpy(np.ascontiguousarray(pairs, np.int32)).to(dev)
    row_off = torch.from_numpy(out_off).to(dev)
    z32 = lambda *shape: torch.zeros(shape, dtype=I32, device=dev)
    bin_cnt, seg_cnt = z32(P, NC), z32(P, NC)
    seg_off = torch.zeros(P * NC + 1, dtype=I64, device=dev)
    pts = torch.empty((max(cap, 1), 4), dtype=torch.float32, device=dev)
    rows = torch.empty((max(cap, 1), 2), dtype=I32, device=dev)
    check(L.iamx_brute_bins(_ptr(idx), _ptr(d2), _ptr(row_off), _ptr(d_pairs), _ptr(kp_off), _ptr(xy),
                            _ptr(size), P, float(match_ratio), float(min_pairs), float(step_d),
                            BRUTE_STEP_A, cap, _ptr(bin_cnt), _ptr(seg_cnt), _ptr(seg_off), _ptr(pts),
                            _ptr(rows), _ptr(flag), stream_ptr()), 'iamx_brute_bins')
    mask, _model, _best, vstatus = verify_pairs(pts[:cap], seg_off, 'homography',
                                                float(tol), hypotheses=hypotheses, seed=seed)
    work = torch.empty(P * (6 * stride + 2 * tab), dtype=I32, device=dev)
    slots = torch.empty((P, stride, 2), dtype=I32, device=dev)
    cnt, chosen, stats, fit_cnt = z32(P), z32(P), z32(P, 4), z32(P, NC)
    off = torch.zeros(P + 1, dtype=I64, device=dev)
    out_rows = torch.empty((max(total, 1), 2), dtype=I32, device=dev)
    check(L.iamx_brute_select(_ptr(d_pairs), _ptr(kp_off), _ptr(key2), P, float(min_pairs), _ptr(seg_cnt),
                              _ptr(seg_off), _ptr(rows), _ptr(mask), _ptr(vstatus), cap, stride, tab,
                              _ptr(work), _ptr(slots), _ptr(cnt), _ptr(off), _ptr(out_rows), total,
                              _ptr(chosen), _ptr(stats), _ptr(fit_cnt), _ptr(flag), stream_ptr()),
          'iamx_brute_select')
    return BruteResult(rows=out_rows, off=off, cnt=cnt, chosen=chosen, stats=stats, fit_cnt=fit_cnt,
                       bin_cnt=bin_cnt, flag=flag, slots=slots, stride=stride)


def brute_pairs(store, pairs, kp_off, xy, size, key2, tol, min_pairs, match_ratio, step_d, hypotheses,
                seed, batch_bytes=BRUTE_BATCH_BYTES):
    dev = require_gpu()
    NC = BRUTE_CELLS
    if not (float(step_d) > 0.0 and math.isfinite(float(step_d))):
        raise ValueError("brute_pairs: step_d must be positive and finite")
    pairs = np.ascontiguousarray(pairs, np.int32).reshape(-1, 2)
    P = len(pairs)
    counts = np.asarray(store.counts, np.int64)
    nq = counts[pairs[:, 0]] if P else np.zeros(0, np.int64)
    ok = (nq >= 2) & (counts[pairs[:, 1]] >= 2) if P else np.zeros(0, bool)
    live = np.nonzero(ok)[0]
    chunks, a = [], 0
    while a < len(live):
        b = a + 1
        while b < len(live) and brute_bytes(nq[live[a:b + 1]]) <= batch_bytes:
            b += 1
        chunks.append(live[a:b])
        a = b
    flag = torch.zeros(2, dtype=I32, device=dev)
    parts = [_brute_launch(store, pairs[c], kp_off, xy, size, key2, tol, min_pairs, match_ratio, step_d,
                           hypotheses, seed, flag) for c in chunks]
    if len(parts) == 1 and len(live) == P:
        return parts[0]
    cnt = torch.zeros(P, dtype=I32, device=dev)
    chosen = torch.full((P,), -1, dtype=I32, device=dev)
    stats = torch.zeros((P, 4), dtype=I32, device=dev)
    stats[:, 1] = -1
    fit_cnt = torch.full((P, NC), -1, dtype=I32, device=dev)
    bin_cnt = torch.zeros((P, NC), dtype=I32, device=dev)
    rows = []
    for c, r in zip(chunks, parts):
        where = torch.from_numpy(c).to(dev)
        cnt[where], chosen[where], stats[where] = r.cnt, r.chosen, r.stats
        fit_cnt[where], bin_cnt[where] = r.fit_cnt, r.bin_cnt
        rows.append(r.rows[:int(r.off[-1])])
    off = exclusive_scan(cnt) if P else torch.zeros(1, dtype=I64, device=dev)
    rows = torch.cat(rows) if rows else torch.empty((0, 2), dtype=I32, device=dev)
    one = len(parts) == 1
    return BruteResult(rows=rows, off=off, cnt=cnt, chosen=chosen, stats=stats, fit_cnt=fit_cnt,
                       bin_cnt=bin_cnt, flag=flag, slots=None, stride=parts[0].stride if one else None)


class PairWorkspace(object):

    def __init__(self, max_rows, max_pairs):
        dev = require_gpu()
        r, p = max(int(max_rows), 1), max(int(max_pairs), 1)
        self.max_rows, self.max_pairs = r, p
        self.idx = torch.empty((r, 2), dtype=I32, device=dev)
        self.d2 = torch.empty((r, 2), dtype=I32, device=dev)
        self.metric = torch.empty(r, dtype=F64, device=dev)
        self.keep = torch.empty(max(r, 8), dtype=U8, device=dev)
        self.seg_count = torch.zeros(p, dtype=I32, device=dev)
        self.surv_off = torch.zeros(p + 1, dtype=I64, device=dev)
        self.surv_q = torch.empty(r, dtype=I32, device=dev)
        self.surv_t = torch.empty(r, dtype=I32, device=dev)
        self.surv_metric = torch.empty(r, dtype=F64, device=dev)
        self.flags = torch.zeros(2, dtype=I32, device=dev)
        self.zero_div = self.flags[0:1]
        self.tile = torch.empty(r, dtype=I32, device=dev)
        self.unresolved = self.flags[1:2]
        self.surv_cnt = torch.zeros(p, dtype=I32, device=dev)
        self.col = self.rowp = self.colmask = self.nar = None
        self.cand_keep = torch.empty(r, dtype=U8, device=dev)
        self.task_total = torch.zeros(2, dtype=I32, device=dev)
        self.tasks = torch.empty((2 * p + r // 32 + 2, 2), dtype=I32, device=dev)

    def ensure_sym(self, col_rows, rowp_rows):
        dev = self.d2.device
        if self.col is None or self.col.shape[0] < col_rows:
            self.col = torch.empty((max(col_rows, 1), 2), dtype=I32, device=dev)
            self.colmask = torch.empty(max(col_rows, 1), dtype=U8, device=dev)
        if self.nar is None:
            self.nar = torch.zeros(max(int(lib().iamx_knn2sym_narrow_bytes(self.max_rows, self.max_pairs)),
                                       256), dtype=U8, device=dev)
        if self.rowp is None or self.rowp.shape[0] < rowp_rows:
            self.rowp = torch.empty((max(rowp_rows, 1), 2), dtype=I32, device=dev)

    def survivor_counts(self, n_pairs):
        first = self.surv_off[:n_pairs].cpu().numpy()
        count = self.surv_cnt[:n_pairs].cpu().numpy().astype(np.int64)
        return first, count

    def survivors(self, n_pairs):
        first, count = self.survivor_counts(n_pairs)
        total = int(self.surv_off[n_pairs].item())
        return (first, count, self.surv_q[:total].cpu().numpy(),
                self.surv_t[:total].cpu().numpy(), self.surv_metric[:total].cpu().numpy())


class UploadArena(object):

    def __init__(self, nbytes=8 << 20, slots=4):
        dev = require_gpu()
        self.dev = dev
        self.slots = [dict(pin=torch.empty(nbytes, dtype=U8).pin_memory(),
                           dev=torch.empty(nbytes, dtype=U8, device=dev),
                           ev=torch.cuda.Event(), used=False) for _ in range(slots)]
        self.cur, self.off, self.k = None, 0, 0

    def begin(self):
        if self.cur is not None:
            self.commit()
        self.k = (self.k + 1) % len(self.slots)
        self.cur = self.slots[self.k]
        if self.cur['used']:
            self.cur['ev'].synchronize()
        self.off = 0

    def put(self, a):
        a = np.ascontiguousarray(a)
        nb = a.nbytes
        off = (self.off + 15) & ~15
        if self.cur is None or off + nb > self.cur['pin'].numel():
            return torch.from_numpy(a).to(self.dev)
        if nb:
            self.cur['pin'].numpy()[off:off + nb] = a.reshape(-1).view(np.uint8)
        self.off = off + nb
        t = self.cur['dev'][off:off + nb].view(_TORCH_OF[a.dtype.str]) if nb else \
            torch.empty(0, dtype=_TORCH_OF[a.dtype.str], device=self.dev)
        return t.view(a.shape) if a.ndim != 1 else t

    def commit(self):
        c = self.cur
        if c is None:
            return
        if self.off:
            c['dev'][:self.off].copy_(c['pin'][:self.off], non_blocking=True)
        c['ev'].record()
        c['used'] = True
        self.cur = None


_TORCH_OF = {'<i4': torch.int32, '<i8': torch.int64, '<f4': torch.float32, '<f8': torch.float64,
             '|u1': torch.uint8, '|i1': torch.int8}


class PairBatch(object):

    def __init__(self, store, pairs, sym=None, arena=None):
        dev = require_gpu()
        up = arena.put if arena is not None else (lambda a: torch.from_numpy(np.ascontiguousarray(a)).to(dev))
        self._up = up
        self.store = store
        pairs = np.ascontiguousarray(pairs, np.int32).reshape(-1, 2)
        counts = np.asarray(store.counts, np.int64)
        self.pairs = pairs
        self.n_pairs = P = len(pairs)
        nq = counts[pairs[:, 0]] if P else np.zeros(0, np.int64)
        if P and counts[pairs[:, 1]].min() < 2:
            raise ValueError("train image with fewer than 2 descriptors")
        self.out_off = np.zeros(P + 1, np.int64)
        np.cumsum(nq, out=self.out_off[1:])
        wg = np.zeros(P + 1, np.int64)
        np.cumsum((nq + 255) // 256, out=wg[1:])
        if wg[-1] >= 2 ** 31:
            raise ValueError("batch too large: split the pair list")
        self.rows = int(self.out_off[-1])
        self.max_query_rows = int(nq.max()) if P else 0
        self.total_wg = int(wg[-1])
        self.d_pairs = up(pairs)
        self.d_wg = up(wg.astype(np.int32))
        self.d_out = up(self.out_off.copy())
        self.fast_rows = 256 if not (P and nq.min() >= 2048) else (1024 if nq.min() >= 4096 else 512)
        wgf = np.zeros(P + 1, np.int64)
        np.cumsum((nq + self.fast_rows - 1) // self.fast_rows, out=wgf[1:])
        self.total_wg_fast = int(wgf[-1])
        self.d_wg_fast = up(wgf.astype(np.int32))
        self.sym = False
        if sym is not False:
            self._setup_sym(dev)
            if sym and not self.sym:
                raise ValueError("symmetric sweep needs both directions of every pair (i != j) "
                                 "in the batch")

    def _setup_sym(self, dev):
        t = sym_tables(self.pairs, self.store.counts, self.store.caps3)
        if t is None:
            return
        assert SYM_ROWS_PER_WG[t['form']] == int(lib().iamx_knn2sym_rows_per_wg(t['form']))
        self.sym = True
        self.sym_form = t['form']
        self.n_u, self.sym_total_wg = len(t['upairs']), int(t['wg'][-1])
        self.sym_col_rows, self.sym_rowp_rows = int(t['col_off'][-1]), int(t['rowp_off'][-1])
        up = self._up
        self.d_upairs = up(np.ascontiguousarray(t['upairs']))
        self.d_sym_wg = up(t['wg'].astype(np.int32))
        self.d_col_off = up(t['col_off'][:-1].copy())
        self.d_rowp_off = up(t['rowp_off'][:-1].copy())
        self.d_osrc = up(t['osrc'])
        self.sym_items_s = t['S']
        self.sym_items_entry = 'iamx_knn2sym_sweep_items16'
        if self.sym_items_s > 1:
            items = sym_items(t['upairs'], self.store.counts, self.sym_items_s)
            self.n_sym_items = len(items)
            self.d_sym_items = up(items)

    def run_sym_sweep(self, ws):
        st = self.store
        ws.ensure_sym(self.sym_col_rows, self.sym_rowp_rows)
        if self.sym_items_s > 1:
            entry = self.sym_items_entry
            check(getattr(lib(), entry)(_ptr(st.desc3), _ptr(st.sn2), _ptr(st.sct), _ptr(st.img_off3),
                                        _ptr(st.img_n), _ptr(self.d_upairs), _ptr(self.d_sym_items),
                                        _ptr(self.d_col_off), _ptr(self.d_rowp_off), self.n_u,
                                        self.n_sym_items, _ptr(ws.col), _ptr(ws.rowp),
                                        _ptr(ws.colmask), stream_ptr()), entry)
            return
        check(lib().iamx_knn2sym_sweep(_ptr(st.desc3), _ptr(st.sn2), _ptr(st.sct), _ptr(st.img_off3),
                                       _ptr(st.img_n), _ptr(self.d_upairs), _ptr(self.d_sym_wg),
                                       _ptr(self.d_col_off), _ptr(self.d_rowp_off), self.n_u,
                                       self.sym_total_wg, self.sym_form, _ptr(ws.col), _ptr(ws.rowp),
                                       _ptr(ws.colmask), stream_ptr()), 'iamx_knn2sym_sweep')

    def run_sym_filter(self, ws, thresh):
        L, s, st = lib(), stream_ptr(), self.store
        check(L.iamx_knn2sym_candidates(_ptr(st.sn2), _ptr(st.sperm), _ptr(st.img_off3), _ptr(st.img_n),
                                        _ptr(self.d_pairs), _ptr(self.d_osrc), _ptr(self.d_sym_wg),
                                        _ptr(self.d_col_off), _ptr(self.d_rowp_off), _ptr(self.d_out),
                                        _ptr(ws.col), _ptr(ws.rowp), self.n_pairs, float(thresh),
                                        _ptr(ws.keep), _ptr(ws.seg_count), _ptr(ws.surv_q),
                                        _ptr(ws.task_total), _ptr(ws.tasks), _ptr(ws.d2),
                                        _ptr(ws.colmask), _ptr(ws.nar), ws.max_rows, self.max_query_rows,
                                        self.sym_form, s),
              'iamx_knn2sym_candidates')
        check(L.iamx_knn2sym_exact(_ptr(st.desc), _ptr(st.norm_q), _ptr(st.norm_t), _ptr(st.key_t),
                                   st.rows_used, _ptr(st.img_off),
                                   _ptr(st.img_n), _ptr(self.d_pairs), _ptr(self.d_out),
                                   _ptr(ws.seg_count), _ptr(ws.task_total), _ptr(ws.tasks),
                                   _ptr(ws.surv_q), self.n_pairs, float(thresh), _ptr(ws.d2),
                                   _ptr(ws.surv_t), _ptr(ws.surv_metric), _ptr(ws.cand_keep),
                                   _ptr(ws.surv_cnt), _ptr(ws.zero_div), _ptr(st.desc3), _ptr(st.sn2),
                                   _ptr(st.sct), _ptr(st.sperm), _ptr(st.img_off3), _ptr(self.d_osrc),
                                   _ptr(ws.nar), ws.max_rows, self.sym_form, s), 'iamx_knn2sym_exact')
        ws.surv_off[:self.n_pairs + 1].copy_(self.d_out, non_blocking=True)

    def run_knn2(self, ws):
        st = self.store
        check(lib().iamx_knn2_l2_pairs(_ptr(st.desc), _ptr(st.norm_q), _ptr(st.norm_t),
                                       _ptr(st.img_off), _ptr(st.img_n), _ptr(self.d_pairs),
                                       _ptr(self.d_wg), _ptr(self.d_out), self.n_pairs,
                                       self.total_wg, _ptr(ws.idx), _ptr(ws.d2), stream_ptr()),
              'iamx_knn2_l2_pairs')

    def _threshold_compact(self, ws, thresh, index, stride, final):
        L, s = lib(), stream_ptr()
        check(L.iamx_match_metric(_ptr(ws.d2), _ptr(self.d_out), self.n_pairs, float(thresh),
                                  _ptr(ws.metric), _ptr(ws.keep), _ptr(ws.seg_count),
                                  _ptr(ws.zero_div), s), 'iamx_match_metric')
        check(L.iamx_exclusive_scan_i32(_ptr(ws.seg_count), self.n_pairs, _ptr(ws.surv_off), s),
              'iamx_exclusive_scan_i32')
        check(L.iamx_match_compact(_ptr(index), stride, _ptr(ws.metric), _ptr(ws.keep),
                                   _ptr(self.d_out), _ptr(ws.surv_off), self.n_pairs,
                                   _ptr(ws.surv_q), _ptr(ws.surv_t), _ptr(ws.surv_metric), s),
              'iamx_match_compact')
        if final:
            ws.surv_cnt[:self.n_pairs].copy_(ws.seg_count[:self.n_pairs])

    def run_filter(self, ws, thresh):
        self._threshold_compact(ws, thresh, ws.idx, 2, True)

    def _route(self, exact_second):
        if self.sym and not exact_second:
            return 'sym'
        if not self.store.has_train_layout:
            return 'general'
        return 'exact' if exact_second else 'bound'

    def run_knn2_fast(self, ws, exact_second=False):
        route = self._route(exact_second)
        if route == 'sym':
            return self.run_sym_sweep(ws)
        if route == 'general':
            return self.run_knn2(ws)
        if route == 'exact' and self.fast_rows == 1024:
            self._use_rows(512)
        st = self.store
        check(lib().iamx_knn2v2_pairs(_ptr(st.desc), _ptr(st.norm_q), _ptr(st.img_off),
                                      _ptr(st.img_n), _ptr(st.desc2), _ptr(st.cinit),
                                      _ptr(st.img_off2), _ptr(st.meta), _ptr(self.d_pairs),
                                      _ptr(self.d_wg_fast), _ptr(self.d_out), self.n_pairs,
                                      self.total_wg_fast, self.fast_rows, 1 if route == 'exact' else 0,
                                      _ptr(ws.d2), _ptr(ws.tile), stream_ptr()),
              'iamx_knn2v2_pairs')

    def _use_rows(self, rows):
        nq = np.asarray(self.store.counts, np.int64)[self.pairs[:, 0]]
        wgf = np.zeros(self.n_pairs + 1, np.int64)
        np.cumsum((nq + rows - 1) // rows, out=wgf[1:])
        self.fast_rows, self.total_wg_fast = rows, int(wgf[-1])
        self.d_wg_fast = torch.from_numpy(wgf.astype(np.int32)).to(self.d_pairs.device)

    def run_filter_fast(self, ws, thresh, exact_second=False):
        route = self._route(exact_second)
        if route == 'sym':
            return self.run_sym_filter(ws, thresh)
        if route == 'general':
            return self.run_filter(ws, thresh)
        L, s, st = lib(), stream_ptr(), self.store
        self._threshold_compact(ws, thresh, ws.tile, 1, route == 'exact')
        if route == 'exact':
            check(L.iamx_knn2v2_resolve(_ptr(st.desc), _ptr(st.norm_q), _ptr(st.img_off),
                                        _ptr(st.desc2), _ptr(st.norm2), _ptr(st.perm),
                                        _ptr(st.img_off2), _ptr(self.d_pairs), _ptr(self.d_out),
                                        _ptr(ws.d2), _ptr(ws.surv_off), _ptr(ws.surv_q),
                                        _ptr(ws.surv_t), self.n_pairs, _ptr(ws.unresolved), s),
                  'iamx_knn2v2_resolve')
        else:
            check(L.iamx_knn2v2_finish(_ptr(st.desc), _ptr(st.norm_q), _ptr(st.img_off),
                                       _ptr(st.desc2), _ptr(st.norm2), _ptr(st.perm),
                                       _ptr(st.img_off2), _ptr(self.d_pairs), _ptr(self.d_out),
                                       _ptr(ws.d2), float(thresh), _ptr(ws.surv_off),
                                       _ptr(ws.surv_q), _ptr(ws.surv_t), _ptr(ws.surv_metric),
                                       _ptr(ws.surv_cnt), self.n_pairs, _ptr(ws.zero_div),
                                       _ptr(ws.unresolved), s), 'iamx_knn2v2_finish')

    def run(self, ws, thresh, fast=True):
        if self.rows > ws.max_rows or self.n_pairs > ws.max_pairs:
            raise ValueError("workspace too small for this batch")
        if self.n_pairs == 0 or self.rows == 0:
            return
        if fast:
            exact = fast == 'exact'
            self.run_knn2_fast(ws, exact_second=exact)
            self.run_filter_fast(ws, thresh, exact_second=exact)
        else:
            self.run_knn2(ws)
            self.run_filter(ws, thresh)


_sift_ws = {}
_sift_out = {}
_prep_ws = {}

DETECT_SLOTS = 8
_slot_tls = threading.local()
_slot_free = None
_slot_lock = threading.Lock()


def _slot_key(dev):
    return (dev.index, getattr(_slot_tls, 'slot', 0))


def wait_stream(polite=None):
    if polite is None:
        polite = getattr(_slot_tls, 'slot', 0) != 0 or getattr(_slot_tls, 'polite', False)
    if not polite:
        torch.cuda.current_stream().synchronize()
        return
    import time
    ev = torch.cuda.Event()
    ev.record()
    pause = 0.0001
    while not ev.query():
        time.sleep(pause)
        pause = min(pause * 1.5, 0.001)


class polite_waits(object):

    def __enter__(self):
        self.prev = getattr(_slot_tls, 'polite', False)
        _slot_tls.polite = True
        return self

    def __exit__(self, *exc):
        _slot_tls.polite = self.prev
        return False


class detector_slot(object):

    def __enter__(self):
        global _slot_free
        with _slot_lock:
            if _slot_free is None:
                import queue
                _slot_free = queue.Queue()
                for k in range(1, DETECT_SLOTS + 1):
                    _slot_free.put(k)
        self.slot = _slot_free.get()
        self.prev = getattr(_slot_tls, 'slot', 0)
        _slot_tls.slot = self.slot
        return self

    def __exit__(self, *exc):
        _slot_tls.slot = self.prev
        _slot_free.put(self.slot)
        return False


class OverlappedSweeps(object):

    def __init__(self, max_rows, max_pairs, first_workspace=None):
        self.ws = [first_workspace or PairWorkspace(max_rows, max_pairs),
                   PairWorkspace(max_rows, max_pairs)]
        self.side = torch.cuda.Stream()
        self.swept = [torch.cuda.Event(), torch.cuda.Event()]
        self.filtered = [torch.cuda.Event(), torch.cuda.Event()]

    def run(self, batches, thresh, after_filter=None, sweep_events=None):
        main = torch.cuda.current_stream()
        for k, b in enumerate(batches):
            w = self.ws[k & 1]
            if k >= 2:
                main.wait_event(self.filtered[k & 1])
            if sweep_events is not None:
                sweep_events[k][0].record()
            b.run_knn2_fast(w)
            if sweep_events is not None:
                sweep_events[k][1].record()
            self.swept[k & 1].record(main)
            self.side.wait_event(self.swept[k & 1])
            with torch.cuda.stream(self.side):
                b.run_filter_fast(w, thresh)
                if after_filter is not None:
                    after_filter(b, w)
                self.filtered[k & 1].record(self.side)
        main.wait_stream(self.side)


def sift_detect(image, cap=200000, contrast_threshold=0.04, edge_threshold=10.0, sigma=1.6,
                order='opencv'):
    dev = require_gpu()
    img = _dev(image, U8)
    if img.dim() == 2:
        h, w, ch = img.shape[0], img.shape[1], 1
    else:
        h, w, ch = img.shape
    need = int(lib().iamx_sift_workspace_bytes(h, w))
    ws = _sift_ws.get(_slot_key(dev))
    if ws is None or ws.numel() < need:
        ws = torch.empty(need, dtype=U8, device=dev)
        _sift_ws[_slot_key(dev)] = ws
    ob = _sift_out.get(_slot_key(dev))
    if ob is None or ob[0].shape[0] < cap:
        ob = (torch.empty((cap, 8), dtype=torch.float32, device=dev),
              torch.empty((cap, 128), dtype=U8, device=dev), torch.zeros(1, dtype=I32, device=dev))
        _sift_out[_slot_key(dev)] = ob
    kp, desc, n = ob[0][:cap], ob[1][:cap], ob[2]
    check(lib().iamx_sift_detect(_ptr(img), h, w, ch, contrast_threshold, edge_threshold, sigma,
                                 _ptr(ws), need, _ptr(kp), _ptr(desc), cap, _ptr(n), stream_ptr()),
          'iamx_sift_detect')
    sw = _sift_sort_ws.get(_slot_key(dev))
    need_s = int(lib().iamx_sift_sort_workspace_bytes(cap))
    if sw is None or sw[0].numel() < need_s or sw[1].shape[0] < cap:
        sw = (torch.empty(need_s, dtype=U8, device=dev),
              torch.empty((cap, 8), dtype=torch.float32, device=dev),
              torch.empty((cap, 128), dtype=U8, device=dev),
              torch.zeros(2, dtype=I32, device=dev))
        _sift_sort_ws[_slot_key(dev)] = sw
    if order not in ('opencv', 'canonical'):
        raise ValueError("sift_detect: order must be 'opencv' or 'canonical'")
    check(lib().iamx_sift_sort(_ptr(kp), _ptr(desc), _ptr(n), cap, 1 if order == 'opencv' else 0,
                               w, h, _ptr(sw[0]), need_s, _ptr(sw[1]), _ptr(sw[2]), _ptr(sw[3]),
                               stream_ptr()), 'iamx_sift_sort')
    sw[3][1:2].copy_(n, non_blocking=True)
    hn = _sift_pinned_count(dev)
    hn.copy_(sw[3], non_blocking=True)
    wait_stream()
    cnt, found = int(hn[0]), int(hn[1])
    if found > cap:
        raise _lib.IamxError("sift_detect: %d keypoints exceed the capacity %d" % (found, cap))
    sift_detect.last_removed = found - cnt
    hk, hd = _sift_pinned(dev, cnt)
    hk[:cnt].copy_(sw[1][:cnt], non_blocking=True)
    hd[:cnt].copy_(sw[2][:cnt], non_blocking=True)
    wait_stream()
    k = hk[:cnt].numpy()
    return k[:, :5].copy(), k[:, 5].copy().view(np.int32), hd[:cnt].numpy().copy()


_sift_sort_ws = {}
_sift_pin = {}


def _sift_pinned_count(dev):
    cur = _sift_pin.get((_slot_key(dev), 'n'))
    if cur is None:
        cur = _sift_pin[(_slot_key(dev), 'n')] = torch.zeros(2, dtype=I32).pin_memory()
    return cur


def _sift_pinned(dev, n):
    cur = _sift_pin.get(_slot_key(dev))
    if cur is None or cur[0].shape[0] < n:
        m = max(1 << 16, 1 << int(n - 1).bit_length())
        cur = (torch.empty((m, 8), dtype=torch.float32).pin_memory(),
               torch.empty((m, 128), dtype=U8).pin_memory())
        _sift_pin[_slot_key(dev)] = cur
    return cur


class JpegCoefficients(object):
    __slots__ = ('info', 'coef', 'quant', '_slot')

    def release(self):
        if self._slot is not None:
            with _jpeg_lock:
                _jpeg_pool.append(self._slot)
            self._slot = None
            self.coef = None


_jpeg_pool = []
_jpeg_lock = __import__('threading').Lock()


# ... 867 lines not shown
```

### include/iamx.h

```cpp
#ifndef IAMX_H
#define IAMX_H

#include <stdint.h>

#ifdef __cplusplus
extern "C" {
#endif

#define IAMX_OK            0
#define IAMX_EINVAL       -1
#define IAMX_ELAUNCH      -2
#define IAMX_ENODEVICE    -3
#define IAMX_EUNSUPPORTED -4
#define IAMX_ENOMEM       -5

#define IAMX_DESC_DIM      128
#define IAMX_ROW_PAD       128

int         iamx_version(void);
const char *iamx_last_error(void);
const char *iamx_arch(void);

int64_t iamx_desc_padded_rows(int64_t n_rows);

int iamx_desc_pack_u8(const uint8_t *src, int64_t n_rows, int8_t *dst,
                      int32_t *norm_q, int32_t *norm_t, void *stream);
int iamx_desc_pack_f32(const float *src, int64_t n_rows, int8_t *dst,
                       int32_t *norm_q, int32_t *norm_t, void *stream);
int iamx_desc_unpack_u8(const int8_t *desc, const int32_t *img_off, const int64_t *dst_off, int n_img,
                        int max_rows_per_image, uint8_t *dst, void *stream);

int iamx_knn2_wg_per_pair(int n_query_rows);

int iamx_knn2_l2_pairs(const int8_t *desc, const int32_t *norm_q, const int32_t *norm_t,
                       const int32_t *img_off, const int32_t *img_n,
                       const int32_t *pairs, const int32_t *wg_off, const int64_t *out_off,
                       int n_pairs, int total_wg,
                       int32_t *out_idx, int32_t *out_d2, void *stream);

int iamx_knn2_l2_u8(const int8_t *q_desc, const int32_t *q_norm_q, int nq,
                    const int8_t *t_desc, const int32_t *t_norm_t, int nt,
                    int32_t *idx, int32_t *d2, void *stream);

int iamx_knn3_l2_pairs(const int8_t *desc, const int32_t *norm_q, const int32_t *norm_t,
                       const int32_t *img_off, const int32_t *img_n,
                       const int32_t *pairs, const int32_t *wg_off, const int64_t *out_off,
                       int n_pairs, int total_wg,
                       int32_t *out_idx, int32_t *out_d2, void *stream);

int iamx_match_metric(const int32_t *d2, const int64_t *seg_off, int n_seg, double thresh,
                      double *metric, uint8_t *keep, int32_t *seg_count, int32_t *zero_div,
                      void *stream);

int iamx_match_compact(const int32_t *idx, int idx_stride, const double *metric,
                       const uint8_t *keep, const int64_t *seg_off, const int64_t *surv_off,
                       int n_seg, int32_t *surv_q, int32_t *surv_t, double *surv_metric,
                       void *stream);

int64_t iamx_desc2_rows_cap(int64_t n_rows);
int iamx_desc2_pack_u8(const uint8_t *src, int64_t n_rows, int8_t *dst, int32_t *norm2,
                       int32_t *cinit, int32_t *perm, int32_t *meta, int32_t *scratch,
                       void *stream);
int iamx_desc2_pack_f32(const float *src, int64_t n_rows, int8_t *dst, int32_t *norm2,
                        int32_t *cinit, int32_t *perm, int32_t *meta, int32_t *scratch,
                        void *stream);
int iamx_desc2_pack_batch_u8(const uint8_t *src, const int64_t *src_off, const int32_t *dst_off,
                             int n_img, int64_t total_rows, int max_rows_per_image, int8_t *dst,
                             int32_t *norm2, int32_t *cinit, int32_t *perm, int32_t *meta,
                             int32_t *scratch, void *stream);
int iamx_knn2v2_pairs(const int8_t *desc_q, const int32_t *norm_q, const int32_t *qimg_off,
                      const int32_t *qimg_n, const int8_t *desc_t, const int32_t *cinit,
                      const int32_t *timg_off, const int32_t *tmeta, const int32_t *pairs,
                      const int32_t *wg_off, const int64_t *out_off, int n_pairs, int total_wg,
                      int rows_per_wg ,
                      int exact_second, int32_t *out_d2, int32_t *out_tile, void *stream);
int iamx_knn2v2_resolve(const int8_t *desc_q, const int32_t *norm_q, const int32_t *qimg_off,
                        const int8_t *desc_t, const int32_t *norm2_t, const int32_t *perm,
                        const int32_t *timg_off, const int32_t *pairs, const int64_t *out_off,
                        const int32_t *d2, const int64_t *surv_off, const int32_t *surv_q,
                        int32_t *surv_t, int n_pairs, int32_t *n_unresolved, void *stream);
int iamx_knn2v2_finish(const int8_t *desc_q, const int32_t *norm_q, const int32_t *qimg_off,
                       const int8_t *desc_t, const int32_t *norm2_t, const int32_t *perm,
                       const int32_t *timg_off, const int32_t *pairs, const int64_t *out_off,
                       int32_t *d2, double thresh, const int64_t *surv_off, int32_t *surv_q,
                       int32_t *surv_t, double *surv_metric, int32_t *surv_cnt, int n_pairs,
                       int32_t *zero_div, int32_t *n_unresolved, void *stream);

int64_t iamx_desc3_rows_cap(int64_t n_rows);
int iamx_knn2sym_rows_per_wg(int form);
const char *iamx_knn2sym_kernel_id(int form);
int iamx_desc3_pack_u8(const uint8_t *src, int64_t n_rows, int8_t *dst, int32_t *sn2,
                       int32_t *sct, int32_t *sperm, int32_t *sinv, int32_t *scratch,
                       void *stream);
int iamx_desc3_pack_f32(const float *src, int64_t n_rows, int8_t *dst, int32_t *sn2,
                        int32_t *sct, int32_t *sperm, int32_t *sinv, int32_t *scratch,
                        void *stream);
int iamx_desc3_pack_batch_u8(const uint8_t *src, const int64_t *src_off, const int32_t *dst_off,
                             int n_img, int64_t total_rows, int max_rows_per_image, int8_t *dst,
                             int32_t *sn2, int32_t *sct, int32_t *sperm, int32_t *sinv,
                             int32_t *scratch, void *stream);
int64_t iamx_knn2sym_narrow_bytes(int64_t rows_total, int n_pairs);
int iamx_knn2sym_sweep(const int8_t *sdesc, const int32_t *sn2, const int32_t *sct,
                       const int32_t *img_off, const int32_t *img_n, const int32_t *upairs,
                       const int32_t *wg_off, const int64_t *col_off, const int64_t *rowp_off,
                       int n_u, int total_wg, int form, int32_t *col, int32_t *rowp,
                       uint8_t *colmask , void *stream);
int iamx_knn2sym_sweep_items(const int8_t *sdesc, const int32_t *sn2, const int32_t *sct,
                             const int32_t *img_off, const int32_t *img_n, const int32_t *upairs,
                             const int32_t *items, const int64_t *col_off, const int64_t *rowp_off,
                             int n_u, int n_items, int32_t *col, int32_t *rowp,
                             uint8_t *colmask , void *stream);
int iamx_knn2sym_sweep_items16(const int8_t *sdesc, const int32_t *sn2, const int32_t *sct,
                               const int32_t *img_off, const int32_t *img_n, const int32_t *upairs,
                               const int32_t *items, const int64_t *col_off, const int64_t *rowp_off,
                               int n_u, int n_items, int32_t *col, int32_t *rowp,
                               uint8_t *colmask , void *stream);
const char *iamx_knn2sym_items16_kernel_id(void);
int iamx_knn2sym_candidates(const int32_t *sn2, const int32_t *sperm, const int32_t *img_off,
                            const int32_t *img_n, const int32_t *pairs, const int32_t *osrc,
                            const int32_t *wg_off, const int64_t *col_off, const int64_t *rowp_off,
                            const int64_t *out_off, const int32_t *col, const int32_t *rowp,
                            int n_pairs, double thresh, uint8_t *keep, int32_t *cand_cnt,
                            int32_t *cand_q, int32_t *task_total, int32_t *tasks, int32_t *d2,
                            const uint8_t *colmask, void *nar , int64_t rows_total,
                            int max_query_rows , int form,
                            void *stream);
int iamx_knn2sym_exact(const int8_t *desc, const int32_t *norm_q, const int32_t *norm_t,
                       int32_t *key_t, int64_t total_rows,
                       const int32_t *img_off, const int32_t *img_n, const int32_t *pairs,
                       const int64_t *out_off, const int32_t *cand_cnt, int32_t *task_total,
                       const int32_t *tasks, int32_t *cand_q, int n_pairs, double thresh,
                       int32_t *d2, int32_t *cand_t, double *cand_metric, uint8_t *cand_keep,
                       int32_t *surv_cnt, int32_t *zero_div, const int8_t *sdesc,
                       const int32_t *sn2, const int32_t *sct, const int32_t *sperm,
                       const int32_t *img_off3, const int32_t *osrc, void *nar ,
                       int64_t rows_total, int form, void *stream);

int iamx_match_postfilter_clip(void);
int iamx_match_pack_results(const int32_t *cnt, const int32_t *status, const int32_t *pairs,
                            const double *z, int n_pairs, int clip, int64_t cap, int64_t *off,
                            int32_t *out_pairs, double *out_z, void *stream);
int iamx_match_postfilter(const int64_t *surv_off, const int32_t *surv_cnt, const int32_t *surv_q,
                          const int32_t *surv_t, const double *surv_metric, const int32_t *pairs,
                          const int64_t *kp_off, const float *xy, const int32_t *key2, int n_pairs,
                          double width, double height, double min_pairs, double threshold_factor,
                          int32_t *out_cnt, int32_t *out_pairs, int32_t *scratch,
                          int32_t *out_stat, int32_t *status, void *stream);

int iamx_thp_pays(void);

int64_t iamx_link_matches(const int32_t *img, const int32_t *kp, const int64_t *ptr,
                          int64_t n_matches, int32_t *out_img, int32_t *out_kp, int64_t *out_ptr,
                          int32_t *n_passes);
int64_t iamx_link_pair_blocks(const int32_t *const *blocks, const int64_t *counts, const int32_t *ij,
                              int64_t n_blocks, int32_t *out_img, int32_t *out_kp, int64_t *out_ptr,
                              int32_t *n_passes);
int iamx_chain_members_uv(const int32_t *f_img, const int32_t *f_kp, int64_t n_members,
                          const float *const *xy, const int64_t *n_kp, int32_t n_images, double *uv,
                          int64_t *bad_member, int threads);
int iamx_kp_key2(const float *xy, int64_t n, int32_t *key2);
int iamx_kp_dup_remap(const float *xy, const uint8_t *used, const int64_t *kp_base, int32_t n_images,
                      int32_t *remap, uint8_t *identity, int threads);
int iamx_match_lists_scan(int32_t *const *lists, const int64_t *cnt, const int32_t *ia,
                          const int32_t *ib, int64_t n_lists, const int64_t *kp_base, int32_t n_images,
                          uint8_t *used, const int32_t *remap, int mode, int32_t *dup_pairs,
                          int32_t *dup_first, int threads);
int iamx_chains_longest_first(const int32_t *img, const int32_t *kp, const int64_t *ptr,
                              int64_t n_chains, int32_t *out_img, int32_t *out_kp, int64_t *out_ptr,
                              int threads);
int iamx_first_occurrence(const int64_t *key, int64_t n, int64_t *first);
int iamx_ledger_index(const int64_t *qi, const int64_t *qj, const int64_t *seq, int64_t m,
                      int64_t n_images, int64_t *other, int64_t *seq_out, int64_t *bounds);
int iamx_pairs_fwd_rev(const int32_t *src, int64_t n, int32_t *fwd, int32_t *rev, int threads);
int iamx_touch_pages(const void *p, int64_t bytes, int threads);
int iamx_segment_mean_std(const double *z, const int64_t *starts, const int64_t *counts,
                          int64_t n_seg, int64_t n_z, double *mean, double *std, int threads);

int iamx_hbm_copy16(const void *src, void *dst, int64_t n16, int reads_per_write, int workgroups,
                    void *stream);

void *iamx_yaw_feedback_new(int n_images, const int32_t *name_rank);
void iamx_yaw_feedback_free(void *h);
int iamx_yaw_feedback_seed(void *h, int image, int n, const int32_t *partner_image, const double *err,
                           const double *weight, const double *dist);
int iamx_yaw_feedback_feed(void *h, int64_t n, const int32_t *pi, const int32_t *pj,
                           const uint8_t *quiet, int64_t n_hits, const int64_t *hit_rows,
                           const double *yv_f, const double *yv_r, const uint8_t *ok, double *e1,
                           double *e2, uint8_t *fresh1, uint8_t *fresh2);
int iamx_yaw_feedback_state(void *h, double *value, uint8_t *touched);

int64_t iamx_group_level(const int32_t *img, const int64_t *ptr, int64_t n_matches, int n_images,
                         int32_t *level, const uint8_t *placed_images, int group_level,
                         int use_single_pairs, int max_wanted, int min_connections,
                         int32_t *placed_matches);
int iamx_triangulate_ground(const double *M, const double *ned, const double *base_elev,
                            int n_images, const int32_t *obs_img, const double *obs_uv,
                            const int64_t *feat_ptr, int64_t n_feat, double *out_ned,
                            int32_t *n_sky, void *stream);

int iamx_triangulate_pairs(const int32_t *pair_img, const double *PROJ, const double *IK,
                           const int64_t *kp_off, const float *xy, const int32_t *m_cnt,
                           const int32_t *m_pairs, int n_pairs, int clip, double *out_z,
                           void *stream);

int iamx_triangulate_pairs_xyz(const int32_t *pair_img, const double *PROJ, const double *IK,
                               const int64_t *kp_off, const float *xy, const int32_t *m_cnt,
                               const int32_t *m_pairs, int n_pairs, int clip, double *out_xyz,
                               void *stream);

int iamx_triangulate_packed(const int32_t *pair_img, const double *pair_proj, const double *IK,
                            const int64_t *kp_off, const float *xy, const int64_t *m_off,
                            const int32_t *m_pairs, int n_pairs, int64_t total, double *out_z,
                            void *stream);

int iamx_similarity_pairs(const int32_t *pair_img, const int64_t *kp_off, const float *xy,
                          const int32_t *m_cnt, const int32_t *m_pairs, int n_pairs, int clip,
                          double *out_aff, int32_t *out_ok, void *stream);

int iamx_exclusive_scan_i32(const int32_t *in, int64_t n, int64_t *out, void *stream);

int iamx_ba_residual(const double *cams, int n_cams, const double *pts, int n_pts,
                     const int32_t *cam_idx, const int32_t *pt_idx, const double *uv,
                     int64_t n_obs, const double *calib, double *r, void *stream);

int iamx_ba_residual_prepared(const double *cams, int n_cams, const double *pts, int n_pts,
                              const int32_t *cam_idx, const int32_t *pt_idx, const double *uv,
                              int64_t n_obs, const double *calib, double *cam_scratch, double *r,
                              void *stream);

int iamx_ba_residual_jac(const double *cams, int n_cams, const double *pts, int n_pts,
                         const int32_t *cam_idx, const int32_t *pt_idx, const double *uv,
                         int64_t n_obs, const double *calib, double *r,
                         double *Jc, double *Jp, double *Jk, void *stream);

int iamx_ba_reproj_stats(const double *cams, int n_cams, const double *pts, int n_pts,
                         const int32_t *cam_idx, const int32_t *pt_idx, const double *uv,
                         int64_t n_obs, const double *calib, const int64_t *cam_ptr,
                         double *cam_stats, double *part, double *summary, double *e,
                         void *stream);

int iamx_ba_mark_outliers(const double *e, int64_t n_obs, double trim_stddev, int has_max,
                          double max_error, double *summary, double *work, int64_t *idx_out,
                          double *e_sel, int64_t cap, void *stream);

int64_t iamx_image_prep_workspace_bytes(int height, int width);
int iamx_image_resized_dims(int height, int width, double scale, int *out_h, int *out_w);
int iamx_image_equalize_resize(const uint8_t *bgr, int height, int width, int equalize,
                               float clip_limit, double scale, void *workspace,
                               int64_t workspace_bytes, uint8_t *out, void *stream);

int iamx_image_prep_stage(int height, int width, int stage, int64_t *offset, int64_t *bytes);

int iamx_image_area_dims(int height, int width, double fx, double fy, int *out_h, int *out_w);
int iamx_image_resize_area(const uint8_t *src, int height, int width, int channels, double fx,
                           double fy, uint8_t *out, void *stream);

int iamx_colour_histogram(const uint8_t *img, int64_t n_pixels, uint32_t *hist, void *stream);
int iamx_colour_accumulate_max_frames(void);
int iamx_colour_accumulate(const uint8_t *const *frames, int n_frames, int64_t n_values, uint32_t *sum,
                           void *stream);
int iamx_colour_mean(const uint32_t *sum, int64_t n_values, int count, uint8_t *avg, void *stream);
int iamx_colour_moments_workspace_doubles(void);
int iamx_colour_moments(const uint8_t *img, int height, int width, double cu, double cv, double *radius,
                        double *partials, double *out, void *stream);
int iamx_colour_fit_mask(int height, int width, double cu, double cv, const double *coef, uint64_t seed,
                         uint8_t *out, void *stream);
int iamx_colour_mask_finish(const uint8_t *img, int64_t n_pixels, uint32_t *chan_max, uint8_t *out,
                            void *stream);
int iamx_colour_lut(const uint8_t *img, int64_t n_pixels, const uint8_t *lut, const uint8_t *mask,
                    uint8_t *out, void *stream);

#define IAMX_SURFACE_RECORD_BYTES 128
#define IAMX_SURFACE_MAX_TRIANGLES (1 << 24)
#define IAMX_SURFACE_MAX_SEED_GRID 4096
#define IAMX_SURFACE_SKY 1
#define IAMX_SURFACE_HIGH_ANGLE 2
#define IAMX_SURFACE_FALLBACK 4
int iamx_surface_pack(const int *simplices, const int *neighbors, const double *transform,
                      int num_triangles, void *records, void *stream);
int iamx_surface_interp(const void *records, int num_triangles, const double *values, int num_points,
                        const int *seed, int seed_g, const double *bbox, const double *xy,
                        int64_t num_queries, int max_steps, double *out, uint8_t *flags, int *steps,
                        void *stream);
int iamx_surface_grid(const void *records, int num_triangles, const double *values, int num_points,
                      const int *seed, int seed_g, const double *bbox, const double *M,
                      const double *ned, const double *avg_ground, int num_images, const double *uv,
                      int num_vertices, int no_extrapolate, int ground_mode, double ground_m,
                      int max_steps, double *pts, int *rounds, uint8_t *flags, int *steps,
                      void *stream);

#define IAMX_TERRAIN_MAX_AXIS 32768
#define IAMX_TERRAIN_SKY 1
#define IAMX_TERRAIN_CAPPED 2
#define IAMX_TERRAIN_LEFT_GRID 4
int iamx_terrain_heights(const double *axis_n, int rows, const double *axis_e, int cols,
                         const double *grid, const double *pts, int64_t num_points, double *z,
                         void *stream);
int iamx_terrain_rays(const double *axis_n, int rows, const double *axis_e, int cols,
                      const double *grid, const double *M, const double *ned, int num_images,
                      const double *uv, int num_rays, double *pts, uint8_t *iters, uint8_t *flags,
                      void *stream);
int iamx_terrain_rays_vec(const double *axis_n, int rows, const double *axis_e, int cols,
                          const double *grid, const double *v, const double *ned, int num_images,
                          int num_rays, double *pts, uint8_t *iters, uint8_t *flags, void *stream);

int64_t iamx_sift_workspace_bytes(int height, int width);
int iamx_sift_detect(const uint8_t *image, int height, int width, int channels,
                     float contrast_threshold, float edge_threshold, float sigma,
                     void *workspace, int64_t workspace_bytes, float *kp, uint8_t *desc, int cap,
                     int32_t *n_out, void *stream);

int iamx_sift_pyramid_level(int height, int width, int octave, int kind, int index,
                            int64_t *byte_offset, int *level_h, int *level_w, int *n_octaves);

int64_t iamx_sift_sort_workspace_bytes(int cap);
int iamx_sift_sort(const float *kp, const uint8_t *desc, const int32_t *n_out, int cap, int order,
                   int width, int height, void *workspace, int64_t workspace_bytes, float *out_kp,
                   uint8_t *out_desc, int32_t *n_sorted, void *stream);

int iamx_jpeg_info(const uint8_t *data, int64_t len, int32_t *info);
int iamx_jpeg_decode_coefficients(const uint8_t *data, int64_t len, int16_t *coef,
                                  int64_t coef_blocks, uint16_t *quant);
int64_t iamx_jpeg_workspace_bytes(const int32_t *info);
int iamx_jpeg_reconstruct(const int16_t *coef, const uint16_t *quant, const int32_t *info,
                          void *workspace, int64_t workspace_bytes, uint8_t *bgr, void *stream);

#define IAMX_JPEG_PENDING     0
#define IAMX_JPEG_SYNCED      1
#define IAMX_JPEG_NOT_SYNCED  2
#define IAMX_JPEG_DAMAGED     3
int64_t iamx_jpeg_entropy_header_bytes(void);
int iamx_jpeg_entropy_prepare(const uint8_t *data, int64_t len, int32_t *info, uint16_t *quant,
                              void *header, int64_t header_bytes);
int64_t iamx_jpeg_entropy_workspace_bytes(const void *header);
int iamx_jpeg_entropy_decode(const uint8_t *data, int64_t data_bytes, const void *header,
                             const void *d_header, void *workspace, int64_t workspace_bytes,
                             int16_t *coef, int64_t coef_blocks, int32_t *status, void *stream);

int64_t iamx_gzip_f32_from_u8_bound(int64_t n_header, int64_t n_values);
int64_t iamx_gzip_f32_from_u8(const uint8_t *header, int64_t n_header, const uint8_t *values,
                              int64_t n_values, uint8_t *out, int64_t out_cap);

int64_t iamx_gzip_members_bound(int64_t total_bytes, int64_t n_members);
int64_t iamx_gzip_members(const uint8_t *const *bufs, const int64_t *lens, int n_bufs,
                          int64_t member_bytes, int level, int strategy, int threads, uint8_t *out,
                          int64_t out_cap);
int64_t iamx_gzip_records_bound(int64_t total, int64_t n_members);
int64_t iamx_gzip_records(const uint8_t *const *bufs, const int64_t *lens, int n_bufs,
                          int64_t member_bytes, int record_bytes, int threads, uint8_t *out,
                          int64_t out_cap);
int iamx_u8_to_f32(const uint8_t *src, float *dst, int64_t n, int threads);
int iamx_f32_to_u8_many(const float *const *srcs, const int64_t *counts, int n, uint8_t *dst,
                        int threads);
int iamx_u8_gather_many(const uint8_t *const *srcs, const int64_t *counts, int n, uint8_t *dst,
                        int threads);
int iamx_feat_records(const float *x, const float *y, const float *size, const float *angle,
                      const float *response, const int32_t *octave, const int32_t *class_id,
                      int64_t n, uint8_t *out);
int64_t iamx_pickle_pair_lists(const int32_t *pairs, const int64_t *off, int64_t n_lists, uint8_t *out,
                               int64_t out_cap, int64_t *out_off);

int iamx_ba_jv(const double *Jc, const double *Jp, const double *Jk, const int32_t *cam_idx,
               const int32_t *pt_idx, int64_t n_obs, int n_cams, int n_pts, const double *x,
               double *y, void *stream);
int iamx_ba_jtv(const double *Jc, const double *Jp, const double *Jk, const int32_t *cam_ptr,
                const int32_t *pt_ptr, const int32_t *pt_obs, int64_t n_obs, int n_cams,
                int n_pts, const double *u, int square, double *out, double *scratch,
                void *stream);

int iamx_ba_lsmr_state_size(void);
int64_t iamx_ba_lsmr_partials_size(int n_cams, int n_pts);
int iamx_ba_lsmr_prepare(const double *cams, const double *pts, const double *d, int n_cams,
                         int n_pts, double *ctab, double *ptab, void *stream);
int iamx_ba_lsmr_iterate(const double *ctab, const double *ptab, const double *calib,
                         const int32_t *pt_idx, const int32_t *cam_ptr, const int32_t *pt_ptr,
                         const int32_t *pt_obs, const int32_t *slot_cp, int64_t n_obs, int n_cams,
                         int n_pts, const double *dreg, double *u1, double *u2, double *vt,
                         double *h, double *hbar, double *x, double *state, double *partials,
                         double *xr, double *tbuf, double *eprod, int n_iter, void *stream);

int iamx_ba_lsmr_phase(const double *ctab, const double *ptab, const double *calib,
                       const int32_t *pt_idx, const int32_t *cam_ptr, const int32_t *pt_ptr,
                       const int32_t *pt_obs, const int32_t *slot_cp, int64_t n_obs, int n_cams,
                       int n_pts, int pt_lo, int pt_hi, const double *dreg, double *u1, double *u2,
                       double *vt, double *h, double *hbar, double *x, double *state,
                       double *partials, double *xr, double *tbuf, double *eprod, int phase,
                       int parity, void *stream);

int iamx_ba_accumulate(const double *Jc, const double *Jp, const double *r, const int32_t *cam_ptr,
                       const int32_t *pt_ptr, const int32_t *pt_obs, int64_t n_obs, int n_cams,
                       int n_pts, double *U, double *V, double *gc, double *gp, void *stream);
int iamx_ba_block_diag(const double *U, const double *V, int n_cams, int n_pts, double *out,
                       void *stream);
int iamx_ba_schur_state_size(void);
int iamx_ba_schur_prepare(const double *Jc, const double *Jp, const double *Jk, const double *r,
                          const int32_t *cam_ptr, const int32_t *pt_idx, int64_t n_obs, int n_cams,
                          int n_pts, const double *V, const double *gp, const double *d,
                          const double *dreg, double *Y, double *yg, double *zp, double *sraw,
                          double *ckpart, void *stream);
int iamx_ba_schur_factor(const double *sraw, const double *d, const double *dreg, int n_cams,
                         int n_pts, int with_calib, double eta, double qtol, int max_iter,
                         double *minv, double *x, double *r, double *z, double *p, double *y,
                         double *state, void *stream);
int iamx_ba_schur_iterate(const double *Jc, const double *Jp, const double *Jk,
                          const int32_t *cam_idx, const int32_t *pt_idx, const int32_t *cam_ptr,
                          const int32_t *pt_ptr, const int32_t *pt_obs, int64_t n_obs, int n_cams,
                          int n_pts, const double *d, const double *dreg, const double *Y,
                          const double *minv, double *t, double *zp, double *qraw, double *part,
                          double *ckpart, double *x, double *r, double *z, double *p, double *y,
                          double *state, int first_iter, int n_iter, int phase, void *stream);
int iamx_ba_schur_finish(const double *Jc, const double *Jp, const double *Jk,
                         const int32_t *cam_idx, const int32_t *pt_ptr, const int32_t *pt_obs,
                         int64_t n_obs, int n_cams, int n_pts, int pt_lo, int pt_hi, const double *d,
                         const double *Y, const double *yg, const double *x, double *y, double *t,
                         double *step, void *stream);

enum { IAMX_LOSS_LINEAR = 0, IAMX_LOSS_HUBER = 1, IAMX_LOSS_SOFT_L1 = 2, IAMX_LOSS_CAUCHY = 3,
       IAMX_LOSS_ARCTAN = 4 };
int iamx_ba_robust_cost(const double *r, int64_t m, int loss, double f_scale, double *out,
                        double *scratch, void *stream);
// ... 267 lines not shown
```

Baseline: 670,000.

## Route per-pair form-2 sweep through the pipelined 16-tile kernel

Moves the knn2sym16 kernel body into a template shared by an ITEMS variant and a per-pair variant, and adds a new iamx_knn2sym_sweep16 entry point. The Python side now sends form-2 sweeps without item splitting to this kernel instead of the older iamx_knn2sym_sweep. The goal is to give plain per-pair launches the deeper staging and scheduling pipeline of the items16 path. The cost is another large specialised kernel that has to match the old sweep's outputs.

New measurement: 671,400, median of 5. About the same (+0.2%).

```diff
diff --git a/imageanalysis_amd/csrc/match_knn2sym.hip b/imageanalysis_amd/csrc/match_knn2sym.hip
--- a/imageanalysis_amd/csrc/match_knn2sym.hip
+++ b/imageanalysis_amd/csrc/match_knn2sym.hip
@@ -976,412 +976,15 @@
 template <int PIPE>
 __global__ __launch_bounds__(256, 1) void knn2sym16_kernel(SymArgs A)
 {
-    constexpr int NW = 4, QB = 16, WGROWS = NW * QB * 16, NT = NW * 64;
-    constexpr int PIECES = CHUNK * D / 16 / NT;
-    constexpr int NT16 = CHUNK / 16, SPT = 4, QS = QB / SPT, NS = NT16 * SPT;
-    static_assert(WGROWS == 1024 && PIECES == 4 && NS == 32 && D == 128, "form 2's workgroup");
-    extern __shared__ __attribute__((aligned(16))) int8_t lds[];
-    int8_t *lds_tile = lds;
-    int *lds_tb = reinterpret_cast<int *>(lds + 2 * CHUNK * D);
-    int *lds_row = lds_tb + 2 * CHUNK;
-    int *lds_cq = lds_row + 3 * NW * CHUNK;
-    int *lds_dump = lds_cq + 2 * NW;
-    const int tid = threadIdx.x, lane = tid & 63, wave = tid >> 6;
-    const int n = lane & 15, lg = lane >> 4;
-    const int rn = ((n & 7) << 1) | (n >> 3);
-
-    int vid;
-    {
-        const int total = A.total_wg, bid = blockIdx.x;
-        const int xcd = bid & 7, k = bid >> 3, q = total >> 3, r = total & 7;
-        vid = (xcd < r ? xcd * (q + 1) : r * (q + 1) + (xcd - r) * q) + k;
-    }
-    int u = A.wg_off[3 * vid], u_end = u + A.wg_off[3 * vid + 1], item_wgi = A.wg_off[3 * vid + 2];
-    v4i bq[QB][2];
-    int fl[4];
-    int bimg_held = -1;
-    asm volatile("" : "+v"(u_end), "+v"(item_wgi), "+v"(bimg_held));
-    const int raw_wave = SWEEP16_LDS_FORM2 + wave * (2 * SWEEP16_RAW_CHUNK);
-    const int raw_wr = raw_wave + lg * SWEEP16_RAW_COMBO + n * 16;
-    const int raw_rd = raw_wave + (lane >> 1) * SWEEP16_RAW_COMBO + (lane & 1) * 16;
-#if defined(IAMX_T_STAMPS)
-    unsigned long long stamp_chunks = 0, stamp_cycles = 0, stamp_ticks = 0, stamp_tail = 0, stamp_c1 = 0;
-#endif
-    int nx_b = A.upairs[2 * u], nx_a = A.upairs[2 * u + 1];
-    int nx_boff = A.img_off[nx_b], nx_nb = A.img_n[nx_b], nx_aoff = A.img_off[nx_a], nx_na = A.img_n[nx_a];
-    int64_t nx_rowp = A.rowp_off[u];
-    for (;;) {
-        const int bimg = uniform32(nx_b);
-        const int boff = uniform32(nx_boff), nb = uniform32(nx_nb);
-        const int aoff = uniform32(nx_aoff), na = uniform32(nx_na);
-        const int capA = (na + CHUNK - 1) / CHUNK * CHUNK;
-        const int nchunks = capA / CHUNK;
-        const int wgi = uniform32(item_wgi);
-        const int q0 = wgi * WGROWS + wave * (QB * 16);
-        const bool wave_valid = q0 < nb;
-        const int64_t rbase = uniform64(nx_rowp) + (int64_t)wgi * capA;
-        if (uniform32(bimg_held) >= 0) __syncthreads();
-
-        if (bimg != uniform32(bimg_held)) {
-            bimg_held = bimg;
-#pragma unroll
-            for (int qb = 0; qb < QB; ++qb) {
-                int row = q0 + QB * rn + qb;
-                row = row < nb ? row : nb - 1;
-                const v4i *src = reinterpret_cast<const v4i *>(A.sdesc + (int64_t)(boff + row) * D);
-#pragma unroll
-                for (int s = 0; s < 2; ++s) {
-                    bq[qb][s] = ~src[4 * s + lg];
-                    asm volatile("" : "+a"(bq[qb][s]));
-                }
-            }
-            {
-                int spread = 0;
-                if (wave_valid) {
-                    const int g_lo = rn & ~1, g_hi = rn | 1;
-                    const int r_lo = q0 + QB * g_lo < nb ? q0 + QB * g_lo : nb - 1;
-                    const int r_hi = q0 + QB * g_hi + QB - 1 < nb ? q0 + QB * g_hi + QB - 1 : nb - 1;
-                    spread = (A.sn2[boff + r_hi] >> 1) - (A.sn2[boff + r_lo] >> 1);
-                }
-#pragma unroll
-                for (int sh = 32; sh >= 1; sh >>= 1) spread = max(spread, __shfl_xor(spread, sh));
-                if (lane == 0) lds_cq[wave] = spread;
-            }
-#pragma unroll
-            for (int j = 0; j < 4; ++j) {
-                const int r_lo = q0 + 2 * QB * (2 * j + (lane & 1));
-                fl[j] = wave_valid ? A.sn2[boff + (r_lo < nb ? r_lo : nb - 1)] >> 1 : 0;
-            }
-        }
-        if (!wave_valid) {
-#pragma unroll
-            for (int k = 0; k < 3 * CHUNK / 64; ++k)
-                lds_row[((k / (CHUNK / 64)) * NW + wave) * CHUNK + (k % (CHUNK / 64)) * 64 + lane] = BIG;
-        }
-        int m[QB][4];
-#pragma unroll
-        for (int qb = 0; qb < QB; ++qb)
-#pragma unroll
-            for (int k = 0; k < 4; ++k) m[qb][k] = BIG;
-
-        const int8_t *tbase = A.sdesc + (int64_t)aoff * D;
-        const int32_t *tci = A.sct + aoff;
-        typedef __attribute__((address_space(3))) void *lds_ptr;
-        auto stage_direct = [&](int ch, int buf) {
-#pragma unroll
-            for (int j = 0; j < PIECES; ++j) {
-                const int e = j * NT + tid, row = e >> 3, slot = (e & 7) ^ ((row >> 1) & 7);
-                const int8_t *gsrc = tbase + (int64_t)(ch * CHUNK + row) * D + slot * 16;
-                int8_t *ldst = lds_tile + buf * (CHUNK * D) + (j * NT + wave * 64) * 16;
-                __builtin_amdgcn_global_load_lds(gsrc, (lds_ptr)ldst, 16, 0, 0);
-            }
-            __builtin_amdgcn_global_load_lds(tci + ch * CHUNK + (tid & (CHUNK - 1)),
-                                             (lds_ptr)(lds_tb + buf * CHUNK + (wave & (CHUNK / 64 - 1)) * 64), 4, 0, 0);
-        };
-        auto wait_direct = [&]() { __builtin_amdgcn_s_waitcnt(0x0F70); };
-        const int mrow = (wave & 1) * 64 + lane;
-        const bool merger = wave < 2;
-        constexpr int RSRC_WORD3_DATA_FORMAT_32 = 4 << 15;
-        constexpr int RANGE_DROP = 0x7FFFFFF0;
-        const __amdgpu_buffer_rsrc_t rowp_rsrc =
-            __builtin_amdgcn_make_buffer_rsrc(A.rowp + 2 * rbase, (short)0, capA * 8, RSRC_WORD3_DATA_FORMAT_32);
-        int spread_w[NW];
-        auto merge_rows = [&](int ch, int rbo, bool store) {
-            int L = BIG, U1 = BIG, U2 = BIG;
-#pragma unroll
-            for (int w = 0; w < NW; ++w) {
-                const int R = lds_row[rbo + w * CHUNK + mrow];
-                const int uw = R + spread_w[w];
-                L = min(L, R);
-                U2 = min(max(U1, uw), U2);
-                U1 = min(U1, uw);
-            }
-            __builtin_amdgcn_raw_buffer_store_b64(v2i{L, pack_row_bounds(L, U1, U2)}, rowp_rsrc,
-                                                  store ? (ch * CHUNK + mrow) * 8 : RANGE_DROP, 0, 0);
-        };
-
-        int *const row_dst = (lane & 1) == 0 && wave_valid
-            ? lds_row + wave * CHUNK + 4 * (lane >> 1)
-            : lds_dump + wave * 256 + 4 * lane;
-        typedef __attribute__((address_space(3))) int8_t *lds_wbytes;
-        typedef __attribute__((address_space(3))) v4i *lds_v4i;
-        auto raw_write = [&](int at, int tile, const int (&rr)[4]) {
-            *reinterpret_cast<lds_v4i>((lds_wbytes)lds + at + tile * (4 * SWEEP16_RAW_COMBO)) = v4i{rr[0], rr[1], rr[2], rr[3]};
-        };
-        auto raw_read = [&](int at, int j, v4i (&v)[2]) {
-#pragma unroll
-            for (int hi = 0; hi < 2; ++hi)
-                v[hi] = *reinterpret_cast<lds_v4i>((lds_wbytes)lds + at + j * 32 + hi * 128);
-        };
-        auto raw_group = [&](int j, const v4i (&v)[2], int (&x)[4]) {
-#pragma unroll
-            for (int i = 0; i < 4; ++i) x[i] = min(v[0][i], v[1][i]) + fl[j];
-        };
-        auto raw_store = [&](int rbo_at, int (&x)[4]) {
-#pragma unroll
-            for (int i = 0; i < 4; ++i) x[i] = min(x[i], __builtin_amdgcn_update_dpp(0, x[i], 0xB1, 0xF, 0xF, true));
-            *reinterpret_cast<v4i *>(row_dst + rbo_at) = v4i{x[0], x[1], x[2], x[3]};
-        };
-        v4i aop[2][2], ct[2];
-        v4i accs[2][QS];
-        int r[2][4];
-#pragma unroll
-        for (int k = 0; k < 4; ++k) r[1][k] = BIG;
-
-        {
-            const int un = u + 1 < u_end ? u + 1 : u;
-            nx_b = A.upairs[2 * un];
-            nx_a = A.upairs[2 * un + 1];
-            nx_rowp = A.rowp_off[un];
-        }
-        stage_direct(0, 0);
-        stage_direct(nchunks > 1 ? 1 : 0, 1);
-        wait_direct();
-        __syncthreads();
-#pragma unroll
-        for (int w = 0; w < NW; ++w) spread_w[w] = __builtin_amdgcn_readfirstlane(lds_cq[w]);
-        {
-            const int b = uniform32(nx_b), a = uniform32(nx_a);
-            nx_boff = A.img_off[b];
-            nx_nb = A.img_n[b];
-            nx_aoff = A.img_off[a];
-            nx_na = A.img_n[a];
-        }
-        typedef __attribute__((address_space(3))) const int8_t *lds_bytes;
-        int opoff[2], tboff = 2 * CHUNK * D + 16 * lg;
-#pragma unroll
-        for (int s = 0; s < 2; ++s) opoff[s] = n * D + (((4 * s + lg) ^ ((n >> 1) & 7)) * 16);
-        auto load_ops = [&](int tile, v4i (&a)[2], v4i &c) {
-            c = *reinterpret_cast<const __attribute__((address_space(3))) v4i *>((lds_bytes)lds + tboff + tile * 64);
-#pragma unroll
-            for (int s = 0; s < 2; ++s)
-                a[s] = *reinterpret_cast<const __attribute__((address_space(3))) v4i *>((lds_bytes)lds + opoff[s] + tile * (16 * D));
-        };
-        auto issue = [&](auto tp_c, auto qp_c, v4i (&acc)[QS]) {
-            constexpr int tp = decltype(tp_c)::value, qp = decltype(qp_c)::value;
-#pragma unroll
-            for (int j = 0; j < QS; ++j) acc[j] = __builtin_amdgcn_mfma_i32_16x16x64_i8(aop[tp][0], bq[qp + j][0], ct[tp], 0, 0, 0);
-#pragma unroll
-            for (int j = 0; j < QS; ++j) acc[j] = __builtin_amdgcn_mfma_i32_16x16x64_i8(aop[tp][1], bq[qp + j][1], acc[j], 0, 0, 0);
-        };
-        load_ops(0, aop[0], ct[0]);
-        load_ops(1, aop[1], ct[1]);
-        issue(int_c<0>{}, int_c<0>{}, accs[0]);
-        __builtin_amdgcn_sched_barrier(0);
-        int rbo = 0, rbo_prev = 2 * NW * CHUNK;
-        const int wave_u = uniform32(wave);
-        const unsigned stage_voff = (unsigned)((tid >> 3) * D + (((tid & 7) ^ ((tid >> 4) & 7)) * 16));
-        const unsigned lds_tile_at = (unsigned)(uintptr_t)(lds_ptr)(lds_tile + wave_u * (64 * 16));
-        const unsigned lds_tb_at = (unsigned)(uintptr_t)(lds_ptr)(lds_tb + (wave_u & (CHUNK / 64 - 1)) * 64);
-        const unsigned ct_voff = (unsigned)((tid & (CHUNK - 1)) * 4);
-#if defined(IAMX_T_STAMPS)
-        const unsigned long long loop_c0 = __builtin_amdgcn_s_memtime(), loop_r0 = __builtin_amdgcn_s_memrealtime();
-        __builtin_amdgcn_s_waitcnt(0xC07F);
-        if (stamp_c1) stamp_tail += loop_c0 - stamp_c1;
-#endif
-        auto chunk = [&](int ch, auto stage_c) __attribute__((always_inline)) {
-            constexpr bool STAGE = decltype(stage_c)::value != 0;
-            const int buf = ch & 1;
-            constexpr int BAR = (NT16 - 2) * SPT;
-            static_assert(BAR + PIECES < NS, "the stage's five pieces fit behind the barrier");
-            const int8_t *const sg_tile = tbase + (int64_t)(ch + 2) * (CHUNK * D);
-            const int8_t *const sg_ct = reinterpret_cast<const int8_t *>(tci + (ch + 2) * CHUNK);
-            const int raw_cur = buf * SWEEP16_RAW_CHUNK, raw_prev = SWEEP16_RAW_CHUNK - raw_cur;
-            const int wr_cur = raw_wr + raw_cur, wr_prev = raw_wr + raw_prev, rd_prev = raw_rd + raw_prev;
-            int mR[NW], mL = BIG, mU1 = BIG, mU2 = BIG;
-            constexpr int RSTORE = 4 * SPT + 1;
-            static_assert(RSTORE < BAR, "the rows are stored in front of the barrier");
-            v4i rdv[2];
-            int racc[4], rx[4], rh[4];
-            static_for<0, NS>([&](auto st_c) {
-                constexpr int st = decltype(st_c)::value;
-                constexpr int t = st / SPT, ph = st % SPT, qp = QS * ph, cur = st & 1, kk = (t >> 1) & 3;
-                constexpr int nst = st + 1 < NS ? st + 1 : 0;
-                constexpr bool staging = STAGE && st >= BAR && st <= BAR + PIECES;
-                if constexpr (st == BAR) {
-                    __builtin_amdgcn_s_waitcnt(0x0070);
-                    __syncthreads();
-                }
-                issue(int_c<(nst / SPT) & 1>{}, int_c<QS * (nst % SPT)>{}, accs[cur ^ 1]);
-#pragma unroll
-                for (int j = 0; j < QS; ++j) {
-                    const v4i &a = accs[cur][j];
-                    int &mm = m[qp + j][kk];
-                    mm = min(min(mm, a[0]), a[1]);
-                    if constexpr (staging) {
-                        if (j == 1) {
-                            if constexpr (st < BAR + PIECES)
-                                stage_piece_held<16>(sg_tile + (st - BAR) * ((NT / 8) * D) + stage_voff,
-                                                     lds_tile_at + buf * (CHUNK * D) + (st - BAR) * NT * 16, mm);
-                            else
-                                stage_piece_held<4>(sg_ct + ct_voff, lds_tb_at + buf * (CHUNK * 4), mm);
-                        }
-                    }
-                    mm = min(min(mm, a[2]), a[3]);
-                }
-                const v4i a0 = accs[cur][0], a1 = accs[cur][1], a2 = accs[cur][2], a3 = accs[cur][3];
-                int (&rc_)[4] = r[t & 1];
-#pragma unroll
-                for (int i = 0; i < 4; ++i)
-                    rc_[i] = ph == 0 ? min(min(min(a0[i], a1[i]), a2[i]), a3[i])
-                                     : min(min(min(min(rc_[i], a0[i]), a1[i]), a2[i]), a3[i]);
-                if constexpr (ph == 0) raw_write(t > 0 ? wr_cur : wr_prev, t > 0 ? t - 1 : NT16 - 1, r[(t + 1) & 1]);
-                if constexpr (ph == 0 && t < 4) raw_read(rd_prev, t, rdv);
-                if constexpr (ph == 2 && t < 4) {
-                    if constexpr (t == 0) raw_group(0, rdv, racc);
-                    else raw_group(t, rdv, rx);
-                    if constexpr (t == 1) {
-#pragma unroll
-                        for (int i = 0; i < 4; ++i) racc[i] = min(racc[i], rx[i]);
-                    }
-                    if constexpr (t == 2) {
-#pragma unroll
-                        for (int i = 0; i < 4; ++i) rh[i] = rx[i];
-                    }
-                    if constexpr (t == 3) {
-#pragma unroll
-                        for (int i = 0; i < 4; ++i) racc[i] = min(min(racc[i], rh[i]), rx[i]);
-                    }
-                }
-                if constexpr (st == RSTORE) raw_store(rbo_prev, racc);
-                if constexpr (ph == SPT - 1) {
-                    if constexpr (t + 2 == NT16) {
-#pragma unroll
-                        for (int s = 0; s < 2; ++s) opoff[s] ^= CHUNK * D;
-                        tboff ^= CHUNK * 4;
-                    }
-                    load_ops((t + 2) % NT16, aop[t & 1], ct[t & 1]);
-                }
-                if constexpr (st == BAR + 1) {
-#pragma unroll
-                    for (int w = 0; w < NW; ++w) mR[w] = lds_row[rbo_prev + w * CHUNK + mrow];
-                }
-                if constexpr (st == BAR + 2) {
-#pragma unroll
-                    for (int w = 0; w < NW; ++w) {
-                        const int uw = mR[w] + spread_w[w];
-                        mL = min(mL, mR[w]);
-                        mU2 = min(max(mU1, uw), mU2);
-                        mU1 = min(mU1, uw);
-                    }
-                    asm volatile("" : "+v"(mL), "+v"(mU1), "+v"(mU2));
-                }
-                if constexpr (st == BAR + 3)
-                    __builtin_amdgcn_raw_buffer_store_b64(v2i{mL, pack_row_bounds(mL, mU1, mU2)}, rowp_rsrc,
-                                                          merger && ch > 0 ? ((ch - 1) * CHUNK + mrow) * 8 : RANGE_DROP, 0, 0);
-                constexpr int nv = 16 + (ph == 2 && t < 4 ? (t & 1 ? 12 : 8) : 0) + (st == RSTORE ? 4 : 0) + (st == 0 ? 3 : 0) +
-                                   (staging ? 2 : 0) + (st == BAR + 2 ? 11 : 0) + (st == BAR + 3 ? 5 : 0) +
-                                   (st == NS - 1 ? 2 : 0) + (PIPE - 2);
-                static_for<0, 8>([&](auto g_c) {
-                    constexpr int g = decltype(g_c)::value;
-                    __builtin_amdgcn_sched_group_barrier(0x008, 1, 0);
-                    __builtin_amdgcn_sched_group_barrier(0x002, sweep16_gap_valu(nv, g) + (g == 7 ? 3 : 0), 0);
-                });
-                __builtin_amdgcn_sched_barrier(0);
-            });
-            rbo_prev = rbo;
-            rbo = rbo == 2 * NW * CHUNK ? 0 : rbo + NW * CHUNK;
-        };
-        int ch = 0;
-        for (; ch + 2 < nchunks; ++ch) chunk(ch, int_c<1>{});
-        for (; ch < nchunks; ++ch) chunk(ch, int_c<0>{});
-#if defined(IAMX_T_STAMPS)
-        {
-            unsigned long long loop_c1;
-            SWEEP_STAMP(loop_c1);
-            stamp_cycles += loop_c1 - loop_c0;
-            stamp_ticks += __builtin_amdgcn_s_memrealtime() - loop_r0;
-            stamp_chunks += (unsigned)nchunks;
-            stamp_c1 = loop_c1;
-            if (A.stamps && lane == 0) {
-                unsigned long long *o = A.stamps + ((size_t)blockIdx.x * NW + wave) * 4;
-                o[0] = stamp_tail;
-                o[1] = stamp_chunks;
-                o[2] = stamp_cycles;
-                o[3] = stamp_ticks;
-            }
-        }
-#endif
-        const int64_t col_v = A.col_off[u];
-        {
-            const int last = ((nchunks - 1) & 1) * SWEEP16_RAW_CHUNK;
-            raw_write(raw_wr + last, NT16 - 1, r[(NT16 - 1) & 1]);
-            v4i v[4][2];
-            int x[4][4];
-#pragma unroll
-            for (int j = 0; j < 4; ++j) raw_read(raw_rd + last, j, v[j]);
-#pragma unroll
-            for (int j = 0; j < 4; ++j) raw_group(j, v[j], x[j]);
-#pragma unroll
-            for (int i = 0; i < 4; ++i) x[0][i] = min(min(x[0][i], x[1][i]), min(x[2][i], x[3][i]));
-            raw_store(rbo_prev, x[0]);
-        }
-        wait_direct();
-        __syncthreads();
-        merge_rows(nchunks - 1, rbo_prev, merger);
-
-        const int64_t col_u = uniform64(col_v);
-        if (wave_valid) {
-            int mk[QB / 2][4], a1[QB / 2], a2[QB / 2];
-#pragma unroll
-            for (int j = 0; j < QB / 2; ++j) {
-#pragma unroll
-                for (int k = 0; k < 4; ++k) {
-                    const v2u x = __builtin_amdgcn_permlane32_swap((unsigned)m[j][k], (unsigned)m[j + QB / 2][k], false, false);
-                    mk[j][k] = min((int)x[0], (int)x[1]);
-                }
-                const int lo01 = min(mk[j][0], mk[j][1]), hi01 = max(mk[j][0], mk[j][1]);
-                const int lo23 = min(mk[j][2], mk[j][3]), hi23 = max(mk[j][2], mk[j][3]);
-                a1[j] = min(lo01, lo23);
-                a2[j] = min(max(lo01, lo23), min(hi01, hi23));
-            }
-            int v1s[4], v2s[4];
-#pragma unroll
-            for (int p = 0; p < 4; ++p) {
-                const v2u x1 = __builtin_amdgcn_permlane16_swap((unsigned)a1[p], (unsigned)a1[p + 4], false, false);
-                const v2u x2 = __builtin_amdgcn_permlane16_swap((unsigned)a2[p], (unsigned)a2[p + 4], false, false);
-                v1s[p] = min((int)x1[0], (int)x1[1]);
-                v2s[p] = min(max((int)x1[0], (int)x1[1]), min((int)x2[0], (int)x2[1]));
-            }
-            const int row0 = q0 + QB * rn + 4 * lg;
-            unsigned maskw = 0;
-            if (A.colmask) {
-                unsigned ownpack = 0;
-#pragma unroll
-                for (int p = 0; p < 4; ++p) {
-                    const v2u w = __builtin_amdgcn_permlane16_swap((unsigned)v2s[p], (unsigned)v2s[p], false, false);
-#pragma unroll
-                    for (int c = 0; c < 2; ++c) {
-                        const int j = p + 4 * c, v2 = (int)w[c];
-                        const unsigned own = (mk[j][0] <= v2 ? 1u : 0u) | (mk[j][1] <= v2 ? 2u : 0u) |
-                                             (mk[j][2] <= v2 ? 4u : 0u) | (mk[j][3] <= v2 ? 8u : 0u);
-                        ownpack |= own << (4 * j);
-                    }
-                }
-                const v2u g = __builtin_amdgcn_permlane16_swap(ownpack, ownpack, false, false);
-                auto spread = [](unsigned nib4) {
-                    const unsigned x = (nib4 | (nib4 << 8)) & 0x00FF00FFu;
-                    return (x | (x << 4)) & 0x0F0F0F0Fu;
-                };
-                const int sh = 16 * (lg & 1);
-                maskw = spread((g[0] >> sh) & 0xFFFFu) | (spread((g[1] >> sh) & 0xFFFFu) << 4);
-            }
-            int32_t *const cdst = A.col + 2 * (col_u + row0);
-            if (row0 + 4 <= nb) {
-                *reinterpret_cast<v4i *>(cdst) = v4i{v1s[0], v2s[0], v1s[1], v2s[1]};
-                *reinterpret_cast<v4i *>(cdst + 4) = v4i{v1s[2], v2s[2], v1s[3], v2s[3]};
-                if (A.colmask) *reinterpret_cast<unsigned *>(A.colmask + col_u + row0) = maskw;
-            } else {
-#pragma unroll
-                for (int p = 0; p < 4; ++p)
-                    if (row0 + p < nb) {
-                        *reinterpret_cast<v2i *>(cdst + 2 * p) = v2i{v1s[p], v2s[p]};
-                        if (A.colmask) A.colmask[col_u + row0 + p] = (uint8_t)(maskw >> (8 * p));
-                    }
-            }
-        }
-        if (++u == uniform32(u_end)) break;
-    }
+    constexpr bool ITEMS = true;
+#include "match_knn2sym16_body.h"
+}
+
+template <int PIPE>
+__global__ __launch_bounds__(256, 1) void knn2sym16_pair_kernel(SymArgs A)
+{
+    constexpr bool ITEMS = false;
+#include "match_knn2sym16_body.h"
 }
 
 struct NarTask { int p, cls, item0, n; };
@@ -2547,6 +2150,20 @@
 }
 
 #define SWEEP16_PIPE 2
+static int sweep16_raise_lds(const void *kernel, int &raised_dev, const char *entry)
+{
+    int dev = 0;
+    if (hipGetDevice(&dev) != hipSuccess)
+        return iamx::fail(IAMX_ELAUNCH, "%s: no current device", entry);
+    if (dev != raised_dev) {
+        const hipError_t e = hipFuncSetAttribute(kernel, hipFuncAttributeMaxDynamicSharedMemorySize, SWEEP16_LDS_BYTES);
+        if (e != hipSuccess)
+            return iamx::fail(IAMX_ELAUNCH, "%s: dynamic LDS: %s", entry, hipGetErrorString(e));
+        raised_dev = dev;
+    }
+    return IAMX_OK;
+}
+
 extern "C" const char *iamx_knn2sym_items16_kernel_id(void)
 {
     return "knn2sym16_kernel<" SWEEP_STR(SWEEP16_PIPE) ">";
@@ -2567,19 +2184,40 @@
     SymArgs a{sdesc, sn2, sct, img_off, img_n, upairs, items, col_off, rowp_off, col, rowp, n_u, n_items,
               colmask SWEEP_STAMPS_ARG};
     static thread_local int raised_dev = -1;
-    int dev = 0;
-    if (hipGetDevice(&dev) != hipSuccess)
-        return iamx::fail(IAMX_ELAUNCH, "iamx_knn2sym_sweep_items16: no current device");
-    if (dev != raised_dev) {
-        const hipError_t e = hipFuncSetAttribute(reinterpret_cast<const void *>(&knn2sym16_kernel<SWEEP16_PIPE>),
-                                                 hipFuncAttributeMaxDynamicSharedMemorySize, SWEEP16_LDS_BYTES);
-        if (e != hipSuccess)
-            return iamx::fail(IAMX_ELAUNCH, "iamx_knn2sym_sweep_items16: dynamic LDS: %s", hipGetErrorString(e));
-        raised_dev = dev;
-    }
+    if (const int rc = sweep16_raise_lds(reinterpret_cast<const void *>(&knn2sym16_kernel<SWEEP16_PIPE>), raised_dev,
+                                         "iamx_knn2sym_sweep_items16"))
+        return rc;
     hipLaunchKernelGGL((knn2sym16_kernel<SWEEP16_PIPE>), dim3((unsigned)n_items), dim3(256), SWEEP16_LDS_BYTES,
                        iamx::as_stream(stream), a);
     return iamx::check_launch("iamx_knn2sym_sweep_items16");
+}
+
+extern "C" const char *iamx_knn2sym_sweep16_kernel_id(void)
+{
+    return "knn2sym16_pair_kernel<" SWEEP_STR(SWEEP16_PIPE) ">";
+}
+
+extern "C" int iamx_knn2sym_sweep16(const int8_t *sdesc, const int32_t *sn2, const int32_t *sct,
+                                    const int32_t *img_off, const int32_t *img_n,
+                                    const int32_t *upairs, const int32_t *wg_off,
+                                    const int64_t *col_off, const int64_t *rowp_off, int n_u,
+                                    int total_wg, int32_t *col, int32_t *rowp, uint8_t *colmask,
+                                    void *stream)
+{
+    IAMX_REQUIRE(sdesc && sn2 && sct && img_off && img_n && upairs && wg_off && col_off && rowp_off &&
+                     col && rowp,
+                 "null pointer");
+    IAMX_REQUIRE(n_u >= 0 && total_wg >= 0, "negative count");
+    if (n_u == 0 || total_wg == 0) return IAMX_OK;
+    SymArgs a{sdesc, sn2, sct, img_off, img_n, upairs, wg_off, col_off, rowp_off, col, rowp, n_u, total_wg,
+              colmask SWEEP_STAMPS_ARG};
+    static thread_local int raised_dev = -1;
+    if (const int rc = sweep16_raise_lds(reinterpret_cast<const void *>(&knn2sym16_pair_kernel<SWEEP16_PIPE>), raised_dev,
+                                         "iamx_knn2sym_sweep16"))
+        return rc;
+    hipLaunchKernelGGL((knn2sym16_pair_kernel<SWEEP16_PIPE>), dim3((unsigned)total_wg), dim3(256), SWEEP16_LDS_BYTES,
+                       iamx::as_stream(stream), a);
+    return iamx::check_launch("iamx_knn2sym_sweep16");
 }
 
 static bool narrow_enabled()
diff --git a/imageanalysis_amd/csrc/match_knn2sym16_body.h b/imageanalysis_amd/csrc/match_knn2sym16_body.h
--- /dev/null
+++ b/imageanalysis_amd/csrc/match_knn2sym16_body.h
@@ -0,0 +1,422 @@
+    constexpr int NW = 4, QB = 16, WGROWS = NW * QB * 16, NT = NW * 64;
+    constexpr int PIECES = CHUNK * D / 16 / NT;
+    constexpr int NT16 = CHUNK / 16, SPT = 4, QS = QB / SPT, NS = NT16 * SPT;
+    static_assert(WGROWS == 1024 && PIECES == 4 && NS == 32 && D == 128, "form 2's workgroup");
+    extern __shared__ __attribute__((aligned(16))) int8_t lds[];
+    int8_t *lds_tile = lds;
+    int *lds_tb = reinterpret_cast<int *>(lds + 2 * CHUNK * D);
+    int *lds_row = lds_tb + 2 * CHUNK;
+    int *lds_cq = lds_row + 3 * NW * CHUNK;
+    int *lds_dump = lds_cq + 2 * NW;
+    const int tid = threadIdx.x, lane = tid & 63, wave = tid >> 6;
+    const int n = lane & 15, lg = lane >> 4;
+    const int rn = ((n & 7) << 1) | (n >> 3);
+
+    int vid;
+    {
+        const int total = A.total_wg, bid = blockIdx.x;
+        const int xcd = bid & 7, k = bid >> 3, q = total >> 3, r = total & 7;
+        vid = (xcd < r ? xcd * (q + 1) : r * (q + 1) + (xcd - r) * q) + k;
+    }
+    int u, u_end, item_wgi;
+    if constexpr (ITEMS) {
+        u = A.wg_off[3 * vid];
+        u_end = u + A.wg_off[3 * vid + 1];
+        item_wgi = A.wg_off[3 * vid + 2];
+    } else {
+        int lo = 0, hi = A.n_u;
+        while (hi - lo > 1) {
+            const int mid = (lo + hi) >> 1;
+            if (A.wg_off[mid] <= vid) lo = mid; else hi = mid;
+        }
+        u = lo;
+        u_end = u + 1;
+        item_wgi = vid - A.wg_off[u];
+    }
+    v4i bq[QB][2];
+    int fl[4];
+    int bimg_held = -1;
+    if constexpr (ITEMS) asm volatile("" : "+v"(u_end), "+v"(item_wgi), "+v"(bimg_held));
+    const int raw_wave = SWEEP16_LDS_FORM2 + wave * (2 * SWEEP16_RAW_CHUNK);
+    const int raw_wr = raw_wave + lg * SWEEP16_RAW_COMBO + n * 16;
+    const int raw_rd = raw_wave + (lane >> 1) * SWEEP16_RAW_COMBO + (lane & 1) * 16;
+#if defined(IAMX_T_STAMPS)
+    unsigned long long stamp_chunks = 0, stamp_cycles = 0, stamp_ticks = 0, stamp_tail = 0, stamp_c1 = 0;
+#endif
+    int nx_b = A.upairs[2 * u], nx_a = A.upairs[2 * u + 1];
+    int nx_boff = A.img_off[nx_b], nx_nb = A.img_n[nx_b], nx_aoff = A.img_off[nx_a], nx_na = A.img_n[nx_a];
+    int64_t nx_rowp = A.rowp_off[u];
+    for (;;) {
+        const int bimg = uniform32(nx_b);
+        const int boff = uniform32(nx_boff), nb = uniform32(nx_nb);
+        const int aoff = uniform32(nx_aoff), na = uniform32(nx_na);
+        const int capA = (na + CHUNK - 1) / CHUNK * CHUNK;
+        const int nchunks = capA / CHUNK;
+        const int wgi = uniform32(item_wgi);
+        const int q0 = wgi * WGROWS + wave * (QB * 16);
+        const bool wave_valid = q0 < nb;
+        const int64_t rbase = uniform64(nx_rowp) + (int64_t)wgi * capA;
+        if constexpr (ITEMS)
+            if (uniform32(bimg_held) >= 0) __syncthreads();
+
+        if (!ITEMS || bimg != uniform32(bimg_held)) {
+            bimg_held = bimg;
+#pragma unroll
+            for (int qb = 0; qb < QB; ++qb) {
+                int row = q0 + QB * rn + qb;
+                row = row < nb ? row : nb - 1;
+                const v4i *src = reinterpret_cast<const v4i *>(A.sdesc + (int64_t)(boff + row) * D);
+#pragma unroll
+                for (int s = 0; s < 2; ++s) {
+                    bq[qb][s] = ~src[4 * s + lg];
+                    asm volatile("" : "+a"(bq[qb][s]));
+                }
+            }
+            {
+                int spread = 0;
+                if (wave_valid) {
+                    const int g_lo = rn & ~1, g_hi = rn | 1;
+                    const int r_lo = q0 + QB * g_lo < nb ? q0 + QB * g_lo : nb - 1;
+                    const int r_hi = q0 + QB * g_hi + QB - 1 < nb ? q0 + QB * g_hi + QB - 1 : nb - 1;
+                    spread = (A.sn2[boff + r_hi] >> 1) - (A.sn2[boff + r_lo] >> 1);
+                }
+#pragma unroll
+                for (int sh = 32; sh >= 1; sh >>= 1) spread = max(spread, __shfl_xor(spread, sh));
+                if (lane == 0) lds_cq[wave] = spread;
+            }
+#pragma unroll
+            for (int j = 0; j < 4; ++j) {
+                const int r_lo = q0 + 2 * QB * (2 * j + (lane & 1));
+                fl[j] = wave_valid ? A.sn2[boff + (r_lo < nb ? r_lo : nb - 1)] >> 1 : 0;
+            }
+        }
+        if (!wave_valid) {
+#pragma unroll
+            for (int k = 0; k < 3 * CHUNK / 64; ++k)
+                lds_row[((k / (CHUNK / 64)) * NW + wave) * CHUNK + (k % (CHUNK / 64)) * 64 + lane] = BIG;
+        }
+        int m[QB][4];
+#pragma unroll
+        for (int qb = 0; qb < QB; ++qb)
+#pragma unroll
+            for (int k = 0; k < 4; ++k) m[qb][k] = BIG;
+
+        const int8_t *tbase = A.sdesc + (int64_t)aoff * D;
+        const int32_t *tci = A.sct + aoff;
+        typedef __attribute__((address_space(3))) void *lds_ptr;
+        auto stage_direct = [&](int ch, int buf) {
+#pragma unroll
+            for (int j = 0; j < PIECES; ++j) {
+                const int e = j * NT + tid, row = e >> 3, slot = (e & 7) ^ ((row >> 1) & 7);
+                const int8_t *gsrc = tbase + (int64_t)(ch * CHUNK + row) * D + slot * 16;
+                int8_t *ldst = lds_tile + buf * (CHUNK * D) + (j * NT + wave * 64) * 16;
+                __builtin_amdgcn_global_load_lds(gsrc, (lds_ptr)ldst, 16, 0, 0);
+            }
+            __builtin_amdgcn_global_load_lds(tci + ch * CHUNK + (tid & (CHUNK - 1)),
+                                             (lds_ptr)(lds_tb + buf * CHUNK + (wave & (CHUNK / 64 - 1)) * 64), 4, 0, 0);
+        };
+        auto wait_direct = [&]() { __builtin_amdgcn_s_waitcnt(0x0F70); };
+        const int mrow = (wave & 1) * 64 + lane;
+        const bool merger = wave < 2;
+        constexpr int RSRC_WORD3_DATA_FORMAT_32 = 4 << 15;
+        constexpr int RANGE_DROP = 0x7FFFFFF0;
+        const __amdgpu_buffer_rsrc_t rowp_rsrc =
+            __builtin_amdgcn_make_buffer_rsrc(A.rowp + 2 * rbase, (short)0, capA * 8, RSRC_WORD3_DATA_FORMAT_32);
+        int spread_w[NW];
+        auto merge_rows = [&](int ch, int rbo, bool store) {
+            int L = BIG, U1 = BIG, U2 = BIG;
+#pragma unroll
+            for (int w = 0; w < NW; ++w) {
+                const int R = lds_row[rbo + w * CHUNK + mrow];
+                const int uw = R + spread_w[w];
+                L = min(L, R);
+                U2 = min(max(U1, uw), U2);
+                U1 = min(U1, uw);
+            }
+            __builtin_amdgcn_raw_buffer_store_b64(v2i{L, pack_row_bounds(L, U1, U2)}, rowp_rsrc,
+                                                  store ? (ch * CHUNK + mrow) * 8 : RANGE_DROP, 0, 0);
+        };
+
+        int *const row_dst = (lane & 1) == 0 && wave_valid
+            ? lds_row + wave * CHUNK + 4 * (lane >> 1)
+            : lds_dump + wave * 256 + 4 * lane;
+        typedef __attribute__((address_space(3))) int8_t *lds_wbytes;
+        typedef __attribute__((address_space(3))) v4i *lds_v4i;
+        auto raw_write = [&](int at, int tile, const int (&rr)[4]) {
+            *reinterpret_cast<lds_v4i>((lds_wbytes)lds + at + tile * (4 * SWEEP16_RAW_COMBO)) = v4i{rr[0], rr[1], rr[2], rr[3]};
+        };
+        auto raw_read = [&](int at, int j, v4i (&v)[2]) {
+#pragma unroll
+            for (int hi = 0; hi < 2; ++hi)
+                v[hi] = *reinterpret_cast<lds_v4i>((lds_wbytes)lds + at + j * 32 + hi * 128);
+        };
+        auto raw_group = [&](int j, const v4i (&v)[2], int (&x)[4]) {
+#pragma unroll
+            for (int i = 0; i < 4; ++i) x[i] = min(v[0][i], v[1][i]) + fl[j];
+        };
+        auto raw_store = [&](int rbo_at, int (&x)[4]) {
+#pragma unroll
+            for (int i = 0; i < 4; ++i) x[i] = min(x[i], __builtin_amdgcn_update_dpp(0, x[i], 0xB1, 0xF, 0xF, true));
+            *reinterpret_cast<v4i *>(row_dst + rbo_at) = v4i{x[0], x[1], x[2], x[3]};
+        };
+        v4i aop[2][2], ct[2];
+        v4i accs[2][QS];
+        int r[2][4];
+#pragma unroll
+        for (int k = 0; k < 4; ++k) r[1][k] = BIG;
+
+        if constexpr (ITEMS) {
+            const int un = u + 1 < u_end ? u + 1 : u;
+            nx_b = A.upairs[2 * un];
+            nx_a = A.upairs[2 * un + 1];
+            nx_rowp = A.rowp_off[un];
+        }
+        stage_direct(0, 0);
+        stage_direct(nchunks > 1 ? 1 : 0, 1);
+        wait_direct();
+        __syncthreads();
+#pragma unroll
+        for (int w = 0; w < NW; ++w) spread_w[w] = __builtin_amdgcn_readfirstlane(lds_cq[w]);
+        if constexpr (ITEMS) {
+            const int b = uniform32(nx_b), a = uniform32(nx_a);
+            nx_boff = A.img_off[b];
+            nx_nb = A.img_n[b];
+            nx_aoff = A.img_off[a];
+            nx_na = A.img_n[a];
+        }
+        typedef __attribute__((address_space(3))) const int8_t *lds_bytes;
+        int opoff[2], tboff = 2 * CHUNK * D + 16 * lg;
+#pragma unroll
+        for (int s = 0; s < 2; ++s) opoff[s] = n * D + (((4 * s + lg) ^ ((n >> 1) & 7)) * 16);
+        auto load_ops = [&](int tile, v4i (&a)[2], v4i &c) {
+            c = *reinterpret_cast<const __attribute__((address_space(3))) v4i *>((lds_bytes)lds + tboff + tile * 64);
+#pragma unroll
+            for (int s = 0; s < 2; ++s)
+                a[s] = *reinterpret_cast<const __attribute__((address_space(3))) v4i *>((lds_bytes)lds + opoff[s] + tile * (16 * D));
+        };
+        auto issue = [&](auto tp_c, auto qp_c, v4i (&acc)[QS]) {
+            constexpr int tp = decltype(tp_c)::value, qp = decltype(qp_c)::value;
+#pragma unroll
+            for (int j = 0; j < QS; ++j) acc[j] = __builtin_amdgcn_mfma_i32_16x16x64_i8(aop[tp][0], bq[qp + j][0], ct[tp], 0, 0, 0);
+#pragma unroll
+            for (int j = 0; j < QS; ++j) acc[j] = __builtin_amdgcn_mfma_i32_16x16x64_i8(aop[tp][1], bq[qp + j][1], acc[j], 0, 0, 0);
+        };
+        load_ops(0, aop[0], ct[0]);
+        load_ops(1, aop[1], ct[1]);
+        issue(int_c<0>{}, int_c<0>{}, accs[0]);
+        __builtin_amdgcn_sched_barrier(0);
+        int rbo = 0, rbo_prev = 2 * NW * CHUNK;
+        const int wave_u = uniform32(wave);
+        const unsigned stage_voff = (unsigned)((tid >> 3) * D + (((tid & 7) ^ ((tid >> 4) & 7)) * 16));
+        const unsigned lds_tile_at = (unsigned)(uintptr_t)(lds_ptr)(lds_tile + wave_u * (64 * 16));
+        const unsigned lds_tb_at = (unsigned)(uintptr_t)(lds_ptr)(lds_tb + (wave_u & (CHUNK / 64 - 1)) * 64);
+        const unsigned ct_voff = (unsigned)((tid & (CHUNK - 1)) * 4);
+#if defined(IAMX_T_STAMPS)
+        const unsigned long long loop_c0 = __builtin_amdgcn_s_memtime(), loop_r0 = __builtin_amdgcn_s_memrealtime();
+        __builtin_amdgcn_s_waitcnt(0xC07F);
+        if (stamp_c1) stamp_tail += loop_c0 - stamp_c1;
+#endif
+        auto chunk = [&](int ch, auto stage_c) __attribute__((always_inline)) {
+            constexpr bool STAGE = decltype(stage_c)::value != 0;
+            const int buf = ch & 1;
+            constexpr int BAR = (NT16 - 2) * SPT;
+            static_assert(BAR + PIECES < NS, "the stage's five pieces fit behind the barrier");
+            const int8_t *const sg_tile = tbase + (int64_t)(ch + 2) * (CHUNK * D);
+            const int8_t *const sg_ct = reinterpret_cast<const int8_t *>(tci + (ch + 2) * CHUNK);
+            const int raw_cur = buf * SWEEP16_RAW_CHUNK, raw_prev = SWEEP16_RAW_CHUNK - raw_cur;
+            const int wr_cur = raw_wr + raw_cur, wr_prev = raw_wr + raw_prev, rd_prev = raw_rd + raw_prev;
+            int mR[NW], mL = BIG, mU1 = BIG, mU2 = BIG;
+            constexpr int RSTORE = 4 * SPT + 1;
+            static_assert(RSTORE < BAR, "the rows are stored in front of the barrier");
+            v4i rdv[2];
+            int racc[4], rx[4], rh[4];
+            static_for<0, NS>([&](auto st_c) {
+                constexpr int st = decltype(st_c)::value;
+                constexpr int t = st / SPT, ph = st % SPT, qp = QS * ph, cur = st & 1, kk = (t >> 1) & 3;
+                constexpr int nst = st + 1 < NS ? st + 1 : 0;
+                constexpr bool staging = STAGE && st >= BAR && st <= BAR + PIECES;
+                if constexpr (st == BAR) {
+                    __builtin_amdgcn_s_waitcnt(0x0070);
+                    __syncthreads();
+                }
+                issue(int_c<(nst / SPT) & 1>{}, int_c<QS * (nst % SPT)>{}, accs[cur ^ 1]);
+#pragma unroll
+                for (int j = 0; j < QS; ++j) {
+                    const v4i &a = accs[cur][j];
+                    int &mm = m[qp + j][kk];
+                    mm = min(min(mm, a[0]), a[1]);
+                    if constexpr (staging) {
+                        if (j == 1) {
+                            if constexpr (st < BAR + PIECES)
+                                stage_piece_held<16>(sg_tile + (st - BAR) * ((NT / 8) * D) + stage_voff,
+                                                     lds_tile_at + buf * (CHUNK * D) + (st - BAR) * NT * 16, mm);
+                            else
+                                stage_piece_held<4>(sg_ct + ct_voff, lds_tb_at + buf * (CHUNK * 4), mm);
+                        }
+                    }
+                    mm = min(min(mm, a[2]), a[3]);
+                }
+                const v4i a0 = accs[cur][0], a1 = accs[cur][1], a2 = accs[cur][2], a3 = accs[cur][3];
+                int (&rc_)[4] = r[t & 1];
+#pragma unroll
+                for (int i = 0; i < 4; ++i)
+                    rc_[i] = ph == 0 ? min(min(min(a0[i], a1[i]), a2[i]), a3[i])
+                                     : min(min(min(min(rc_[i], a0[i]), a1[i]), a2[i]), a3[i]);
+                if constexpr (ph == 0) raw_write(t > 0 ? wr_cur : wr_prev, t > 0 ? t - 1 : NT16 - 1, r[(t + 1) & 1]);
+                if constexpr (ph == 0 && t < 4) raw_read(rd_prev, t, rdv);
+                if constexpr (ph == 2 && t < 4) {
+                    if constexpr (t == 0) raw_group(0, rdv, racc);
+                    else raw_group(t, rdv, rx);
+                    if constexpr (t == 1) {
+#pragma unroll
+                        for (int i = 0; i < 4; ++i) racc[i] = min(racc[i], rx[i]);
+                    }
+                    if constexpr (t == 2) {
+#pragma unroll
+                        for (int i = 0; i < 4; ++i) rh[i] = rx[i];
+                    }
+                    if constexpr (t == 3) {
+#pragma unroll
+                        for (int i = 0; i < 4; ++i) racc[i] = min(min(racc[i], rh[i]), rx[i]);
+                    }
+                }
+                if constexpr (st == RSTORE) raw_store(rbo_prev, racc);
+                if constexpr (ph == SPT - 1) {
+                    if constexpr (t + 2 == NT16) {
+#pragma unroll
+                        for (int s = 0; s < 2; ++s) opoff[s] ^= CHUNK * D;
+                        tboff ^= CHUNK * 4;
+                    }
+                    load_ops((t + 2) % NT16, aop[t & 1], ct[t & 1]);
+                }
+                if constexpr (st == BAR + 1) {
+#pragma unroll
+                    for (int w = 0; w < NW; ++w) mR[w] = lds_row[rbo_prev + w * CHUNK + mrow];
+                }
+                if constexpr (st == BAR + 2) {
+#pragma unroll
+                    for (int w = 0; w < NW; ++w) {
+                        const int uw = mR[w] + spread_w[w];
+                        mL = min(mL, mR[w]);
+                        mU2 = min(max(mU1, uw), mU2);
+                        mU1 = min(mU1, uw);
+                    }
+                    asm volatile("" : "+v"(mL), "+v"(mU1), "+v"(mU2));
+                }
+                if constexpr (st == BAR + 3)
+                    __builtin_amdgcn_raw_buffer_store_b64(v2i{mL, pack_row_bounds(mL, mU1, mU2)}, rowp_rsrc,
+                                                          merger && ch > 0 ? ((ch - 1) * CHUNK + mrow) * 8 : RANGE_DROP, 0, 0);
+                constexpr int nv = 16 + (ph == 2 && t < 4 ? (t & 1 ? 12 : 8) : 0) + (st == RSTORE ? 4 : 0) + (st == 0 ? 3 : 0) +
+                                   (staging ? 2 : 0) + (st == BAR + 2 ? 11 : 0) + (st == BAR + 3 ? 5 : 0) +
+                                   (st == NS - 1 ? 2 : 0) + (PIPE - 2);
+                static_for<0, 8>([&](auto g_c) {
+                    constexpr int g = decltype(g_c)::value;
+                    __builtin_amdgcn_sched_group_barrier(0x008, 1, 0);
+                    __builtin_amdgcn_sched_group_barrier(0x002, sweep16_gap_valu(nv, g) + (g == 7 ? 3 : 0), 0);
+                });
+                __builtin_amdgcn_sched_barrier(0);
+            });
+            rbo_prev = rbo;
+            rbo = rbo == 2 * NW * CHUNK ? 0 : rbo + NW * CHUNK;
+        };
+        int ch = 0;
+        for (; ch + 2 < nchunks; ++ch) chunk(ch, int_c<1>{});
+        for (; ch < nchunks; ++ch) chunk(ch, int_c<0>{});
+#if defined(IAMX_T_STAMPS)
+        {
+            unsigned long long loop_c1;
+            SWEEP_STAMP(loop_c1);
+            stamp_cycles += loop_c1 - loop_c0;
+            stamp_ticks += __builtin_amdgcn_s_memrealtime() - loop_r0;
+            stamp_chunks += (unsigned)nchunks;
+            stamp_c1 = loop_c1;
+            if (A.stamps && lane == 0) {
+                unsigned long long *o = A.stamps + ((size_t)blockIdx.x * NW + wave) * 4;
+                o[0] = stamp_tail;
+                o[1] = stamp_chunks;
+                o[2] = stamp_cycles;
+                o[3] = stamp_ticks;
+            }
+        }
+#endif
+        const int64_t col_v = A.col_off[u];
+        {
+            const int last = ((nchunks - 1) & 1) * SWEEP16_RAW_CHUNK;
+            raw_write(raw_wr + last, NT16 - 1, r[(NT16 - 1) & 1]);
+            v4i v[4][2];
+            int x[4][4];
+#pragma unroll
+            for (int j = 0; j < 4; ++j) raw_read(raw_rd + last, j, v[j]);
+#pragma unroll
+            for (int j = 0; j < 4; ++j) raw_group(j, v[j], x[j]);
+#pragma unroll
+            for (int i = 0; i < 4; ++i) x[0][i] = min(min(x[0][i], x[1][i]), min(x[2][i], x[3][i]));
+            raw_store(rbo_prev, x[0]);
+        }
+        wait_direct();
+        __syncthreads();
+        merge_rows(nchunks - 1, rbo_prev, merger);
+
+        const int64_t col_u = uniform64(col_v);
+        if (wave_valid) {
+            int mk[QB / 2][4], a1[QB / 2], a2[QB / 2];
+#pragma unroll
+            for (int j = 0; j < QB / 2; ++j) {
+#pragma unroll
+                for (int k = 0; k < 4; ++k) {
+                    const v2u x = __builtin_amdgcn_permlane32_swap((unsigned)m[j][k], (unsigned)m[j + QB / 2][k], false, false);
+                    mk[j][k] = min((int)x[0], (int)x[1]);
+                }
+                const int lo01 = min(mk[j][0], mk[j][1]), hi01 = max(mk[j][0], mk[j][1]);
+                const int lo23 = min(mk[j][2], mk[j][3]), hi23 = max(mk[j][2], mk[j][3]);
+                a1[j] = min(lo01, lo23);
+                a2[j] = min(max(lo01, lo23), min(hi01, hi23));
+            }
+            int v1s[4], v2s[4];
+#pragma unroll
+            for (int p = 0; p < 4; ++p) {
+                const v2u x1 = __builtin_amdgcn_permlane16_swap((unsigned)a1[p], (unsigned)a1[p + 4], false, false);
+                const v2u x2 = __builtin_amdgcn_permlane16_swap((unsigned)a2[p], (unsigned)a2[p + 4], false, false);
+                v1s[p] = min((int)x1[0], (int)x1[1]);
+                v2s[p] = min(max((int)x1[0], (int)x1[1]), min((int)x2[0], (int)x2[1]));
+            }
+            const int row0 = q0 + QB * rn + 4 * lg;
+            unsigned maskw = 0;
+            if (A.colmask) {
+                unsigned ownpack = 0;
+#pragma unroll
+                for (int p = 0; p < 4; ++p) {
+                    const v2u w = __builtin_amdgcn_permlane16_swap((unsigned)v2s[p], (unsigned)v2s[p], false, false);
+#pragma unroll
+                    for (int c = 0; c < 2; ++c) {
+                        const int j = p + 4 * c, v2 = (int)w[c];
+                        const unsigned own = (mk[j][0] <= v2 ? 1u : 0u) | (mk[j][1] <= v2 ? 2u : 0u) |
+                                             (mk[j][2] <= v2 ? 4u : 0u) | (mk[j][3] <= v2 ? 8u : 0u);
+                        ownpack |= own << (4 * j);
+                    }
+                }
+                const v2u g = __builtin_amdgcn_permlane16_swap(ownpack, ownpack, false, false);
+                auto spread = [](unsigned nib4) {
+                    const unsigned x = (nib4 | (nib4 << 8)) & 0x00FF00FFu;
+                    return (x | (x << 4)) & 0x0F0F0F0Fu;
+                };
+                const int sh = 16 * (lg & 1);
+                maskw = spread((g[0] >> sh) & 0xFFFFu) | (spread((g[1] >> sh) & 0xFFFFu) << 4);
+            }
+            int32_t *const cdst = A.col + 2 * (col_u + row0);
+            if (row0 + 4 <= nb) {
+                *reinterpret_cast<v4i *>(cdst) = v4i{v1s[0], v2s[0], v1s[1], v2s[1]};
+                *reinterpret_cast<v4i *>(cdst + 4) = v4i{v1s[2], v2s[2], v1s[3], v2s[3]};
+                if (A.colmask) *reinterpret_cast<unsigned *>(A.colmask + col_u + row0) = maskw;
+            } else {
+#pragma unroll
+                for (int p = 0; p < 4; ++p)
+                    if (row0 + p < nb) {
+                        *reinterpret_cast<v2i *>(cdst + 2 * p) = v2i{v1s[p], v2s[p]};
+                        if (A.colmask) A.colmask[col_u + row0 + p] = (uint8_t)(maskw >> (8 * p));
+                    }
+            }
+        }
+        if constexpr (!ITEMS) break;
+        else if (++u == uniform32(u_end)) break;
+    }
diff --git a/imageanalysis_amd/kernels.py b/imageanalysis_amd/kernels.py
--- a/imageanalysis_amd/kernels.py
+++ b/imageanalysis_amd/kernels.py
@@ -1080,6 +1080,7 @@
         self.d_osrc = up(t['osrc'])
         self.sym_items_s = t['S']
         self.sym_items_entry = 'iamx_knn2sym_sweep_items16'
+        self.sym_pair_entry = 'iamx_knn2sym_sweep16'
         if self.sym_items_s > 1:
             items = sym_items(t['upairs'], self.store.counts, self.sym_items_s)
             self.n_sym_items = len(items)
@@ -1094,6 +1095,14 @@
                                         _ptr(st.img_n), _ptr(self.d_upairs), _ptr(self.d_sym_items),
                                         _ptr(self.d_col_off), _ptr(self.d_rowp_off), self.n_u,
                                         self.n_sym_items, _ptr(ws.col), _ptr(ws.rowp),
+                                        _ptr(ws.colmask), stream_ptr()), entry)
+            return
+        if self.sym_form == 2 and self.sym_pair_entry != 'iamx_knn2sym_sweep':
+            entry = self.sym_pair_entry
+            check(getattr(lib(), entry)(_ptr(st.desc3), _ptr(st.sn2), _ptr(st.sct), _ptr(st.img_off3),
+                                        _ptr(st.img_n), _ptr(self.d_upairs), _ptr(self.d_sym_wg),
+                                        _ptr(self.d_col_off), _ptr(self.d_rowp_off), self.n_u,
+                                        self.sym_total_wg, _ptr(ws.col), _ptr(ws.rowp),
                                         _ptr(ws.colmask), stream_ptr()), entry)
             return
         check(lib().iamx_knn2sym_sweep(_ptr(st.desc3), _ptr(st.sn2), _ptr(st.sct), _ptr(st.img_off3),
diff --git a/include/iamx.h b/include/iamx.h
--- a/include/iamx.h
+++ b/include/iamx.h
@@ -116,6 +116,12 @@
                                int n_u, int n_items, int32_t *col, int32_t *rowp,
                                uint8_t *colmask , void *stream);
 const char *iamx_knn2sym_items16_kernel_id(void);
+int iamx_knn2sym_sweep16(const int8_t *sdesc, const int32_t *sn2, const int32_t *sct,
+                         const int32_t *img_off, const int32_t *img_n, const int32_t *upairs,
+                         const int32_t *wg_off, const int64_t *col_off, const int64_t *rowp_off,
+                         int n_u, int total_wg, int32_t *col, int32_t *rowp,
+                         uint8_t *colmask , void *stream);
+const char *iamx_knn2sym_sweep16_kernel_id(void);
 int iamx_knn2sym_candidates(const int32_t *sn2, const int32_t *sperm, const int32_t *img_off,
                             const int32_t *img_n, const int32_t *pairs, const int32_t *osrc,
                             const int32_t *wg_off, const int64_t *col_off, const int64_t *rowp_off,
```
